# Huiweizhou/GCGCN

Measured on AMD Instinct MI355X. Metric: docs/sec fwd+bwd through CAGGC+MAGGC, higher is better.
Workload: dtype f32; 1 GPU; c2: GraphHops fwd+bwd, B=32/GPU N=64 D=256 L=2 H=8, train mode, E1/E2/X/params require grad, rotating inputs: 3 resident batches (805 MB of E per GPU), step i runs on batch i mod 3; global_batch=32, mode=graph, input_sets=3, parallelism=dp1, grad_allreduce=one coalesced collective after backward

## Files before the change

gcgcn_amd/_lib.py:

```python
from __future__ import annotations

import ctypes
import os
from ctypes import c_char_p, c_float, c_int, c_int64, c_uint64, c_void_p

_HERE = os.path.dirname(os.path.abspath(__file__))
LIB_PATH = os.environ.get("GCGCN_LIB") or os.path.join(_HERE, "lib", "libgcgcn_hip.so")

ABI_VERSION = 7

SALT_GAT = 0x47415431
SALT_MHA = 0x4D484131
SALT_GCN = 0x47434E31
SALT_GLUE = 0x474C5531

P = c_void_p
I = c_int
F = c_float
L = c_int64

class MhaHook(ctypes.Structure):
    _fields_ = [("flat_q", c_void_p), ("Q", c_void_p), ("P", c_void_p), ("A", c_void_p), ("dQ", c_void_p), ("rng_snap", c_void_p),
                ("p", ctypes.c_float)]


class EdgeRide(ctypes.Structure):
    _fields_ = [("B", ctypes.c_int32), ("N", ctypes.c_int32), ("D", ctypes.c_int32),
                ("inp", c_void_p), ("n_valid", c_void_p), ("out", c_void_p)]


SIGNATURES = {
    "gcgcn_version": (I, []),
    "gcgcn_last_error": (c_char_p, []),
    "gcgcn_set_option": (I, [c_char_p, I]),
    "gcgcn_debug_spread": (I, [L, L, L, L, P, P]),
    "gcgcn_debug_chain_plan": (I, [I] * 11 + [P]),
    "gcgcn_debug_head_plan": (I, [I, I, I, I, P]),
    "gcgcn_debug_gemm_plan": (I, [I, P, P, I, L, L, P]),
    "gcgcn_debug_edge_plan": (I, [I] * 13 + [P]),
    "gcgcn_debug_attn_plan": (I, [I] * 8 + [P]),
    "gcgcn_debug_out_bwd_plan": (I, [I] * 12 + [P]),
    "gcgcn_prof_start": (I, [c_char_p, I]),
    "gcgcn_prof_enable": (I, [I]),
    "gcgcn_prof_stop": (I, [P, P, P]),
    "gcgcn_rng_next": (I, [P, P, I, P]),
    "gcgcn_dropout_keep": (I, [P, L, P, c_uint64, F, P]),
    "gcgcn_dropout": (I, [P, P, L, P, c_uint64, F, P]),
    "gcgcn_gat_layout": (I, [I, I, P]),
    "gcgcn_gat_fwd": (I, [I, I, I, I, P, P, P, P, P, F, P, P, P, P, P, P, P, I, P, I, P]),
    "gcgcn_gat_bwd_scratch": (L, [I, I, I]),
    "gcgcn_gat_bwd": (I, [I, I, I, I, P, P, P, P, P, F, P, P, P, P, P, P, P, P, P, P, P, P, P, P, P]),
    "gcgcn_edge_mean_fwd": (I, [I, I, I, P, P, P, P]),
    "gcgcn_edge_mean_bwd": (I, [I, I, I, P, P, P, P]),
    "gcgcn_mha_layout": (I, [I, P]),
    "gcgcn_mha_scratch": (L, [I, I, I]),
    "gcgcn_row_blocks_ints": (L, [I, I]),
    "gcgcn_row_blocks": (I, [I, I, P, P, P]),
    "gcgcn_mha_fwd": (I, [I, I, I, I, P, P, P, P, F, P, P, P, P, P, P]),
    "gcgcn_mha_bwd": (I, [I, I, I, I, P, P, P, F, P, P, P, P, P, P, P, P, P, P, I, P, P]),
    "gcgcn_maggc_fusable": (I, [I, I, I]),
    "gcgcn_gcn_layout": (I, [I, I, I, P]),
    "gcgcn_gcn_scratch": (L, [I, I, I, I]),
    "gcgcn_gcn_fwd": (I, [I, I, I, I, I, P, P, P, P, P, P, F, P, F, P, P, P, P, P, P, P, P, P, P, P, P]),
    "gcgcn_gcn_bwd": (I, [I, I, I, I, I, P, P, P, P, P, P, F, P, F, P, P, P, P, P, P, P, P, P, P, P, P, P, P, P, P, P, P, P, P, P, P]),
    "gcgcn_defer_create": (P, []),
    "gcgcn_defer_destroy": (None, [P]),
    "gcgcn_defer_count": (I, [P]),
    "gcgcn_defer_flush": (I, [P, P]),
    "gcgcn_graphconv_fwd": (I, [I, I, I, I, I, P, P, P, P, P, P, P, P, P, P, P]),
    "gcgcn_graphconv_bwd": (I, [I, I, I, I, I, P, P, P, P, P, P, P, P, P, P, P, P, P, P, P, P, P, P, P, P]),
    "gcgcn_pair_bce_fwd": (I, [I, I, I, P, P, P, P, P, P]),
    "gcgcn_pair_bce_bwd": (I, [I, I, I, P, P, P, P, P, P]),
    "gcgcn_eval_ws_bytes": (L, [L, L]),
    "gcgcn_eval_scan": (I, [I, I, I, P, P, P, P, P, P, L, P, P]),
    "gcgcn_eval_rank": (I, [P, L, P, L, P, P]),
    "gcgcn_eval_curve": (I, [P, L, L, P, ctypes.c_double, P, P, P, P, P, L, P]),
    "gcgcn_producer_layout": (I, [I, I, P]),
    "gcgcn_producer_count": (I, [I, I, I, I, P, P, P, P]),
    "gcgcn_producer_sizes": (I, [I, I, I, I, I, I, I, L, L, P]),
    "gcgcn_producer_fwd": (I, [I, I, I, I, I, I, I, P, P, P, P, I, P, P, P, P, L, L, P, P, P, L, P, P]),
    "gcgcn_producer_bwd": (I, [I, I, I, I, I, I, I, P, P, P, P, I, P, P, P, P, L, L, P, P, P, P, P, P, P, P, P, P]),
    "gcgcn_edge_mean_fwd_compact": (I, [I, I, I, P, P, P, P, P, P]),
    "gcgcn_edge_mean_bwd_compact": (I, [I, I, I, P, P, P, P, P, P, P]),
    "gcgcn_gat_fwd_compact": (I, [I, I, I, I, P, P, P, P, P, P, P, F, P, P, P, P, P, P, P, I, I, P]),
    "gcgcn_gat_bwd_compact_scratch": (L, [I, I, I]),
    "gcgcn_gat_bwd_compact": (I, [I, I, I, I, P, P, P, P, P, P, P, F, P, P, P, P, P, P, P, P, P, P, P, P, P, P, P]),
    "gcgcn_head_layout": (I, [I, I, I, I, I, P]),
    "gcgcn_head_sizes": (I, [I, I, I, I, P]),
    "gcgcn_head_fwd": (I, [I, I, I, I, I, I, I, I, I, P, P, P, P, P, P, P, P, P, P, P]),
    "gcgcn_head_bwd": (I, [I, I, I, I, I, I, I, I, I, P, P, P, P, P, P, P, P, P, P, P, P, P, P, P, P]),
    "gcgcn_tensorise": (I, [I, I, I, I, I, I, I, P, I, P, I, P, I, P, P, P, P, P, P, P, P, P, P, P, P]),
    "gcgcn_adam_step": (I, [I, P, L, ctypes.c_double, ctypes.c_double, ctypes.c_double, P]),
    "gcgcn_adam_ws_bytes": (L, [I, L]),
    "gcgcn_adam_step_dev": (I, [I, P, L, ctypes.c_double, ctypes.c_double, ctypes.c_double, P, ctypes.c_double, P, L, P, P]),
    "gcgcn_gemm": (I, [I, I, I, P, L, I, P, L, I, P, L, I, L, L, L, F, P, I, I, I, I, P, L, P]),
    "gcgcn_gemm_dyn": (I, [I, I, I, P, L, I, P, L, I, P, L, P, I, P, I, L, P, L, P]),
    "gcgcn_lstm_ws_bytes": (L, [I] * 5),
    "gcgcn_lstm_fwd": (I, [I] * 5 + [P] * 10),
    "gcgcn_lstm_bwd": (I, [I] * 5 + [P] * 17 + [L, P]),
    "gcgcn_frontend_ws_bytes": (L, [I] * 9),
    "gcgcn_embed_fwd": (I, [I] * 8 + [P] * 9),
    "gcgcn_embed_bwd": (I, [I] * 8 + [P] * 5 + [I, I] + [P] * 4 + [L, P]),
    "gcgcn_context_fwd": (I, [I] * 5 + [P] * 8),
    "gcgcn_context_bwd": (I, [I] * 5 + [P] * 11 + [L, P]),
}

_lib = None


def lib() -> ctypes.CDLL:
    global _lib
    if _lib is None:
        if not os.path.exists(LIB_PATH):
            raise RuntimeError(
                f"gcgcn_amd: {LIB_PATH} not found. Build it with `make -C gcgcn_amd/csrc` "
                "(or `python -c 'import __graft_entry__ as g; g.build()'`). There is no CPU fallback.")
        handle = ctypes.CDLL(LIB_PATH)
        for name, (res, args) in SIGNATURES.items():
            fn = getattr(handle, name)
            fn.restype = res
            fn.argtypes = args
        if handle.gcgcn_version() != ABI_VERSION:
            raise RuntimeError(f"gcgcn_amd: ABI version {handle.gcgcn_version()} != {ABI_VERSION}")
        _lib = handle
    return _lib


def call(name: str, *args):
    h = lib()
    rc = getattr(h, name)(*args)
    if rc != 0:
        raise RuntimeError(f"{name} failed ({rc}): {h.gcgcn_last_error().decode()}")


def layout(kind: str, *dims) -> list:
    n = {"gat": 9, "mha": 3, "gcn": 7, "producer": 17, "head": 7}[kind]
    out = (c_int64 * n)()
    call(f"gcgcn_{kind}_layout", *dims, ctypes.cast(out, c_void_p))
    return list(out)
```

gcgcn_amd/csrc/api.hip:

```cpp
#include "../../include/gcgcn.h"

#include <stdarg.h>
#include <string.h>

#include <new>
#include <vector>

#include <stdlib.h>

#include "attn_plan.hpp"
#include "compact.hpp"
#include "gat_body.hpp"
#include "gemm.hpp"
#include "lstm.hpp"
#include "frontend.hpp"
#include "rowops.hpp"

namespace gc {

static thread_local char g_err[512] = "";

void set_error(const char* fmt, ...) {
  va_list ap;
  va_start(ap, fmt);
// ... 102 lines not shown
      o.value = value, o.resolved = true;
      return true;
    }
  return false;
}

static AttnQuery make_attn_query(int N, int D, int H, const void* Q, const void* dQ, bool hook, bool chain_attends, bool core_done) {
  return AttnQuery{N, D, H, attn_misalign(Q, dQ), hook, chain_attends, core_done, option("mha_core", 1)};
}

static int make_ride(const char* who, const gcgcn_edge_ride* ride, int kind, EdgeRide& r) {
  memset(&r, 0, sizeof(r));
  if (!ride) return 0;
  GC_REQUIRE(ride->B > 0 && ride->N > 0 && ride->D > 0 && ride->in && ride->out, "%s: bad edge ride B=%d N=%d D=%d", who,
             ride->B, ride->N, ride->D);
  GC_REQUIRE((long)ride->B * ride->N <= 0x3fffffffL, "%s: edge ride too large", who);
  r.kind = kind, r.B = ride->B, r.N = ride->N, r.D = ride->D;
  r.in = ride->in, r.n_valid = ride->n_valid, r.out = ride->out;
  return 0;
}

static void use_rows(GemmArgs& g, const int* rowblk, int mode, int zero_dead = 0) {
  if (!rowblk) return;
  g.rb = rowblk + ROWBLK_HDR, g.rb_n = rowblk;
  g.rb_mode = mode, g.rb_zero = zero_dead;
}

static const int* live_rows(const int32_t* rowblk, int N, bool ragged) {
  return (rowblk && ragged && N % 16 == 0 && N >= 32) ? rowblk : nullptr;
}

static ChainQuery make_query(int B, int N, int D, int L, int H, const GcnLayout& y, const float* flat, bool ragged, bool scratch,
                             bool hook, const EdgeRide& ride, const void* A, const void* Pn, const void* Y) {
  ChainQuery q = ChainQuery();
  q.B = B, q.N = N, q.D = D, q.L = L, q.H = H, q.gh = y.gh;
  q.HD = (long)H * D, q.oWd = y.oWd, q.wd_head = y.wd_head, q.oWlin = y.oWlin;
  q.flat = flat, q.ragged = ragged, q.scratch = scratch, q.hook = hook, q.ride = ride;
  q.A = A, q.Pn = Pn, q.Y = Y;
  q.chain = option("chain", 1), q.chain_big = option("chain_big", 0), q.chain_t = option("chain_t", 1);
  return q;
}

static GcnCtx make_ctx(int B, int N, int D, int L, int H, const GcnLayout& y, const float* X, const float* A,
                       const float* flat, const int* n_valid, Drop drop) {
  GcnCtx c;
  memset(&c, 0, sizeof(c));
  c.B = B, c.N = N, c.D = D, c.L = L, c.H = H, c.gh = y.gh;
  c.HD = (long)H * D, c.oWd = y.oWd, c.wd_head = y.wd_head;
  c.X = X, c.A = A, c.flat = flat, c.n_valid = n_valid, c.drop = drop;
  return c;
}

struct EdgeOperand {
  const float* E;
  CmpE ce;
};

static int gat_node_fwd(const float* X, const float* flat, float* uvc, float* s, long M, int D, int Dh, int uvc_valid, void* rng_state,
                        void* rng_snaps, int rng_count, hipStream_t st) {
  if (!uvc_valid) {
    GC_TRY(gat_fold_fwd(flat, uvc, D, Dh, st, rng_state, rng_snaps, rng_count));
    return node_score_fwd(X, uvc, s, M, D, st);
  }
  return node_score_fwd(X, uvc, s, M, D, st, rng_state, rng_snaps, rng_count);
}

static int gat_bwd(const EdgeOperand& eo, int B, int N, int D, int Dh, const float* X, const int* n_valid, const float* flat, Drop drop,
                   const float* uvc, const float* P, const float* dA, const float* dEbar, const float* dX_in, float* dX, float* dE,
                   float* dbias, float* dflat, float* dlogit, float* ds, float* dvpart, float* duvc, float* scratch, DeferQueue* dq,
                   hipStream_t st) {
  const bool compact = eo.E == nullptr;
  const long M = (long)B * N;
  const float* v = uvc + D;
  const EdgePlan plan = edge_plan_bwd({B, N, D, compact, true, dE != nullptr, dEbar != nullptr,
                                       compact ? 0u : edge_misalign(eo.E, v, dE, dEbar, nullptr)});
  const GatTail tail{P, dA, uvc, dX_in, ds, dX, drop, B, plan.slices};
  if (plan.route == EdgePlan::ONE) {
    GC_TRY(gat_dlogit(P, dA, uvc, dX_in, dlogit, ds, dX, B, N, D, plan.slices, drop, st));
  } else if (plan.route == EdgePlan::THREE) {
    GC_TRY(softmax_bwd(P, dA, dlogit, M, N, drop, st));
    GC_TRY(colsum(dlogit, nullptr, ds, N, N, N, B, (long)N * N, 0, N, 0, nullptr, st));
    GC_TRY(node_score_bwd(ds, uvc, dX_in, dX, M, D, st));
  }
  if (compact)
    GC_TRY(cmp_bwd(eo.ce, v, n_valid, dlogit, dEbar, dE, dvpart, scratch + plan.rowbuf_off, dbias, plan, B, N, D, st));
  else
    GC_TRY(edge_bwd(eo.E, v, n_valid, dlogit, dEbar, dE, dvpart, plan, B, N, D, st, dq, &tail));
  long part_off[3];
  int ns = 0;
  GC_TRY(colsum3(X, ds, duvc, M, D, D, dvpart, nullptr, duvc + D, M, D, D, ds, nullptr, duvc + 2 * D, M, 1, 1, scratch,
                 st, false, part_off, &ns));
  return gat_fold_bwd(flat, duvc, dflat, D, Dh, st, scratch, part_off, ns);
}

static OutBwdPlan out_bwd_plan(const OutBwdQuery& q) {
  OutBwdPlan p = OutBwdPlan();
  const bool masked = q.ragged || q.odrop;
  if (q.fuse) {
    p.mask = masked ? OutBwdPlan::MASK_CHAIN : OutBwdPlan::MASK_NONE;
    p.wsum = q.H == 1 ? OutBwdPlan::WSUM_NONE : q.wsum_fwd ? OutBwdPlan::WSUM_FORWARD : OutBwdPlan::WSUM_HERE;
    p.dwlin = OutBwdPlan::DWLIN_BACK;
    const bool in_chain = 2 * q.B <= COL_RIDE_SLICES;
    p.col1 = in_chain ? OutBwdPlan::COL1_CHAIN : OutBwdPlan::COL1_BACK;
    p.chain_slices = in_chain ? 2 * q.B : 0;
    return p;
  }
  p.mask = masked ? OutBwdPlan::MASK_LAUNCH : OutBwdPlan::MASK_NONE;
  constexpr long fold_max = 2L << 20;
  const bool fold = q.scratch && (q.H == 1 || q.wsum_fwd) && (long)q.B * q.N * q.H * q.D <= fold_max && q.dxres_aligned;
  p.fold = !fold ? OutBwdPlan::FOLD_NONE : q.H == 1 ? OutBwdPlan::FOLD_ONE_HEAD : OutBwdPlan::FOLD_HEADS;
  p.fold_drop = fold && (q.H == 1 || q.drop);
  p.head_sum_launch = !fold;
  p.wsum = p.fold == OutBwdPlan::FOLD_HEADS ? OutBwdPlan::WSUM_FORWARD : OutBwdPlan::WSUM_NONE;
  p.dwlin = OutBwdPlan::DWLIN_FRONT;
  p.col1 = q.scratch ? OutBwdPlan::COL1_FRONT : OutBwdPlan::COL1_OWN_LAUNCH;
  return p;
}

static OutBwdCol2 out_bwd_plan_col2(const OutBwdPlan& p, bool front_reduced) {
  switch (p.col1) {
    case OutBwdPlan::COL1_OWN_LAUNCH: return {OutBwdCol2::DONE, 0};
    case OutBwdPlan::COL1_CHAIN: return {OutBwdCol2::BACK_LAUNCH, p.chain_slices};
    case OutBwdPlan::COL1_BACK: return {OutBwdCol2::BACK_REDUCE, 0};
    default: break;
  }
  if (front_reduced) return {OutBwdCol2::FRONT_REDUCE, 0};
  if (p.head_sum_launch) return {OutBwdCol2::HEAD_SUM_KERNEL, 0};
  return {OutBwdCol2::BACK_LAUNCH, COL_RIDE_SLICES};
}

}

using namespace gc;

extern "C" {

int gcgcn_version(void) { return 7; }
const char* gcgcn_last_error(void) { return g_err; }

int gcgcn_set_option(const char* name, int value) {
  GC_REQUIRE(name, "set_option: null name");
  if (set_opt(name, value)) return 0;
  set_error("set_option: unknown option '%s'", name);
  return 1;
}

int64_t gcgcn_row_blocks_ints(int B, int N) { return (B > 0 && N > 0 && N % 16 == 0) ? row_blocks_ints(B, N) : 0; }
int gcgcn_row_blocks(int B, int N, const int32_t* n_valid, int32_t* out, void* stream) {
  return row_blocks(n_valid, B, N, out, (hipStream_t)stream);
}

int gcgcn_prof_start(const char* kernel_prefix, int capacity) {
  GC_REQUIRE(kernel_prefix && capacity > 0, "prof_start: bad arguments");
  for (hipEvent_t e : g_prof.ev) (void)hipEventDestroy(e);
  g_prof.ev.assign(2 * (size_t)capacity, nullptr);
  for (auto& e : g_prof.ev) {
    if (hipEventCreate(&e) != hipSuccess) {
      set_error("prof_start: hipEventCreate failed");
      return 2;
    }
  }
  strncpy(g_prof.filter, kernel_prefix, sizeof(g_prof.filter) - 1);
  g_prof.used = 0;
  g_prof.work = 0;
  g_prof.on = true;
  return 0;
}
int gcgcn_prof_enable(int on) {
  g_prof.on = on != 0 && !g_prof.ev.empty();
  return 0;
}
int gcgcn_prof_stop(double* total_ms, int* launches, double* work) {
  GC_REQUIRE(total_ms && launches, "prof_stop: null pointer");
  if (work) *work = g_prof.work;
// ... 136 lines not shown
  o[2] = o[1] + D;
  return 0;
}

int gcgcn_mha_fwd(int B, int N, int D, int H, const float* X, const int32_t* n_valid, const float* flat,
                  const void* rng_snap, float p, float* Q, float* P, float* A, float* scratch, const int32_t* rowblk, void* stream) {
  hipStream_t st = (hipStream_t)stream;
  GC_TRY(check_dims("mha_fwd", B, N, D, 1, H));
  const long wse = scratch ? gemm_scratch_elems(B, N, D, 1) : 0;
  GC_REQUIRE(X && flat && Q && P, "mha_fwd: null pointer");
  const AttnPlan plan = attn_plan_fwd(make_attn_query(N, D, H, Q, nullptr, false, false, false));
  const GcnCtx::MhaFwd m = attn_core(GcnCtx::MhaFwd{Q, P, A}, D, H, plan, rng_snap, p);
  GC_REQUIRE(!m.drop.snap || A, "mha_fwd: dropout on but A is NULL");
  const long M = (long)B * N;
  {
    GemmArgs g = gemm_nt(X, D, flat, D, Q, D, (int)M, D, D).split_ws(scratch, wse);
    g.bias = flat + (long)D * D;
    use_rows(g, live_rows(rowblk, N, n_valid != nullptr), 1, 1);
    GC_TRY(gemm(g, st));
  }
  switch (plan.route) {
    case AttnPlan::CORE: return mha_core_fwd(m, n_valid, B, N, D, H, st);
    default: {
      GemmArgs g = gemm_nt(Q, D, Q, D, P, N, N, N, m.dh).split_ws(scratch, wse);
      g.batch_z1(B, (long)N * D, (long)N * D, (long)H * N * N).batch_z2(H, m.dh, m.dh, (long)N * N);
      g.alpha = m.alpha;
      GC_TRY(gemm(g, st));
      return softmax_fwd(P, nullptr, n_valid, P, A, M * H, N, H, m.drop, st);
    }
  }
}

int64_t gcgcn_mha_scratch(int B, int N, int D) { return scratch_elems(B, N, D, 1); }

int gcgcn_mha_bwd(int B, int N, int D, int H, const float* X, const float* flat, const void* rng_snap, float p,
                  const float* Q, const float* P, const float* dA, const float* dX_in, float* dX, float* dflat, float* dS,
                  float* dQ, float* scratch, void* defer_queue, int core_done, const int32_t* rowblk, void* stream) {
  hipStream_t st = (hipStream_t)stream;
  GC_TRY(check_dims("mha_bwd", B, N, D, 1, H));
  const long wse = scratch ? gemm_scratch_elems(B, N, D, 1) : 0;
  GC_REQUIRE(X && flat && Q && P && dA && dX && dflat && dS && dQ, "mha_bwd: null pointer");
  const AttnPlan plan = attn_plan_bwd(make_attn_query(N, D, H, Q, dQ, false, false, core_done != 0));
  const MhaPass mp = attn_core(mha_pass(Q, P, dA, dQ, B, N, D, H), D, H, plan, rng_snap, p);
  const long M = (long)B * N;
  switch (plan.route) {
    case AttnPlan::DONE: break;
    case AttnPlan::CORE: GC_TRY(mha_core_bwd(mp, st)); break;
    default:
      GC_TRY(softmax_bwd(P, dA, dS, M * H, N, mp.drop, st));
      for (int pass = 0; pass < 2; ++pass) {
        GemmArgs g = (pass == 0 ? gemm_nn : gemm_tn)(dS, N, Q, D, dQ, D, N, mp.dh, N).split_ws(scratch, wse);
        g.batch_z1(B, (long)H * N * N, (long)N * D, (long)N * D).batch_z2(H, (long)N * N, mp.dh, mp.dh);
        g.alpha = mp.alpha, g.accumulate = pass;
        GC_TRY(gemm(g, st));
      }
  }
  {
    GemmArgs gs[2] = {gemm_nn(dQ, D, flat, D, dX, D, (int)M, D, D).split_ws(scratch, wse),
                      gemm_tn(dQ, D, X, D, dflat, D, D, D, (int)M).split_ws(scratch, wse)};
    gs[0].add = dX_in, gs[0].ldadd = D;
    const int* rows = live_rows(rowblk, N, true);
    use_rows(gs[0], rows, 1, 1), use_rows(gs[1], rows, 2);
    const int ng = gemm_defer((DeferQueue*)defer_queue, gs[1]) ? 1 : 2;
    if (scratch) {
      const ColRide cr = col_sum(dQ, M, D, D, dflat + (long)D * D, scratch + wse);
      bool later = false;
      GC_TRY(gemm_group(gs, ng, st, &cr, (ng == 1 && defer_queue) ? &later : nullptr));
      if (later) {
        const ColRide c2 = cr.stage2(COL_RIDE_SLICES);
        if (!gemm_defer_col2((DeferQueue*)defer_queue, c2)) GC_TRY(col_sum_stage2_launch(c2, st));
      }
    } else {
      GC_TRY(gemm_group(gs, ng, st));
      GC_TRY(colsum(dQ, nullptr, dflat + (long)D * D, M, D, D, 1, 0, 0, 0, 0, scratch, st));
    }
  }
  return 0;
}

void* gcgcn_defer_create(void) { return new (std::nothrow) DeferQueue(); }
void gcgcn_defer_destroy(void* queue) { delete (DeferQueue*)queue; }
int gcgcn_defer_count(const void* queue) { return queue ? ((const DeferQueue*)queue)->n + ((const DeferQueue*)queue)->ncol2 : 0; }
int gcgcn_defer_flush(void* queue, void* stream) { return gemm_flush_deferred((DeferQueue*)queue, (hipStream_t)stream); }

int gcgcn_pair_bce_fwd(int B, int N, int R, const float* logits, const float* labels, const int32_t* n_valid, float* loss,
                       float* part, void* stream) {
  GC_REQUIRE(B > 0 && N > 0 && R > 0 && (long)B * N <= 0x7fffffffL && (long)N * R <= 0x7fffffffL,
             "pair_bce_fwd: bad shape B=%d N=%d R=%d", B, N, R);
  GC_REQUIRE(logits && labels && loss && part, "pair_bce_fwd: null pointer");
  return pair_bce_fwd(logits, labels, n_valid, loss, part, B, N, R, (hipStream_t)stream);
}

int gcgcn_pair_bce_bwd(int B, int N, int R, const float* logits, const float* labels, const int32_t* n_valid,
                       const float* dloss, float* dlogits, void* stream) {
  GC_REQUIRE(B > 0 && N > 0 && R > 0, "pair_bce_bwd: bad shape B=%d N=%d R=%d", B, N, R);
  GC_REQUIRE(logits && labels && dlogits, "pair_bce_bwd: null pointer");
  return pair_bce_bwd(logits, labels, n_valid, dloss, dlogits, B, N, R, (hipStream_t)stream);
}

int gcgcn_gcn_layout(int D, int L, int H, int64_t* o) {
  GC_TRY(check_dims("gcn_layout", 1, 1, D, L, H));
  GC_REQUIRE(o, "gcn_layout: null pointer");
  const GcnLayout y = gcn_layout(D, L, H);
  o[0] = y.oWnX, o[1] = y.oWe, o[2] = y.oWd, o[3] = y.oWlin, o[4] = y.oblin, o[5] = y.total, o[6] = y.wd_head;
  return 0;
}

int gcgcn_gcn_fwd(int B, int N, int D, int L, int H, const float* X, const float* Ebar, const float* A,
                  const int32_t* n_valid, const float* flat, const void* rng_snap, float p, const void* out_rng_snap,
                  float out_p, float* out, float* Pn, float* Y, float* HO, float* rinv, float* G, float* wsum, float* scratch,
                  const gcgcn_edge_ride* ride, const gcgcn_mha_hook* mha, const int32_t* rowblk, void* stream) {
  hipStream_t st = (hipStream_t)stream;
  GC_TRY(check_dims("gcn_fwd", B, N, D, L, H));
  AttnQuery aq = make_attn_query(N, D, H, mha ? mha->Q : nullptr, nullptr, mha != nullptr, false, false);
  const int refusal = attn_hook_refusal(aq);
  GC_REQUIRE(refusal != ATTN_REFUSED_SHAPE, "gcn_fwd: attention hook on a shape it does not serve");
  GC_REQUIRE(!mha || (mha->flat_q && mha->Q && mha->P), "gcn_fwd: attention hook on a shape it does not serve");
  GC_REQUIRE(refusal != ATTN_REFUSED_ALIGN, "gcn_fwd: attention hook: misaligned Q");
  if (mha) A = mha->A ? mha->A : mha->P;
  EdgeRide er;
  GC_TRY(make_ride("gcn_fwd", ride, 1, er));
  const long wse = scratch ? gemm_scratch_elems(B, N, D, H) : 0;
  GC_REQUIRE(X && Ebar && A && flat && out && Pn && Y && HO && rinv && G, "gcn_fwd: null pointer");
  const GcnLayout y = gcn_layout(D, L, H);
  const Drop drop = make_drop(rng_snap, GCGCN_SALT_GCN, p);
  const long M = (long)B * N;
  const long HD = (long)H * D;
  GC_REQUIRE(M <= 0x7fffffffL, "gcn_fwd: B*N too large");
  ChainQuery q = make_query(B, N, D, L, H, y, flat, n_valid != nullptr, scratch != nullptr, mha != nullptr, er, A, Pn, Y);
  q.G = G, q.HO = HO, q.X = X;
  const ChainPlan plan = chain_plan_fwd(q);
  aq.chain_attends = plan.attention;
  const AttnPlan ap = attn_plan_fwd(aq);
  GcnCtx c = make_ctx(B, N, D, L, H, y, X, A, flat, n_valid, drop);
  c.G = G, c.Pn = Pn, c.Y = Y, c.HO = HO, c.rinv = rinv;
  if (plan.ride) c.ride = er;
  const int* rows = live_rows(rowblk, N, n_valid != nullptr);

  {
    GemmArgs g3[3] = {gemm_nn(X, D, flat + y.oWnX, HD, Pn, HD, (int)M, (int)HD, D).split_ws(scratch, wse),
                      gemm_nn(Ebar, D, flat + y.oWe, HD, G, HD, (int)M, (int)HD, D).split_ws(scratch, wse), GemmArgs()};
    const int ng = mha ? 3 : 2;
    if (mha) {
      g3[2] = gemm_nt(X, D, mha->flat_q, D, mha->Q, D, (int)M, D, D).split_ws(scratch, wse);
      g3[2].bias = mha->flat_q + (long)D * D;
    }
    for (int q = 0; q < ng; ++q) use_rows(g3[q], rows, 1, 1);
    const ColRide hs = head_sum(flat + y.oWlin, H, D, wsum);
    GC_TRY(gemm_group(g3, ng, st, (wsum && H > 1) ? &hs : nullptr));
  }
  {
    if (er.kind && !plan.ride) {
      GC_TRY(edge_fwd(er.in, nullptr, er.n_valid, er.out, nullptr, nullptr, nullptr, Drop(), er.B, er.N, er.D, st));
      er.kind = 0;
    }
    if (mha) {
      const GcnCtx::MhaFwd m = attn_core(GcnCtx::MhaFwd{mha->Q, mha->P, mha->A}, D, H, ap, mha->rng_snap, mha->p);
      GC_REQUIRE(!m.drop.snap || mha->A, "gcn_fwd: attention dropout on but A is NULL");
      switch (ap.route) {
        case AttnPlan::CHAIN: c.mha = m; break;
        default: GC_TRY(mha_core_fwd(m, n_valid, B, N, D, H, st));
      }
    }
    if (plan.kind != ChainPlan::NONE) {
      GC_TRY(gcn_chain_fwd(c, plan, st));
    } else {
// ... 206 lines not shown
    GemmArgs g = gemm_tn(A, N, dS, Dout, dT, Dout, N, Dout, N).batch_z1(B, (long)N * N, (long)N * Dout, (long)N * Dout);
    GC_TRY(gemm(g, st, 0, 1));
  }
  GemmArgs gs[5] = {
      gemm_nt(dS, Dout, T, Dout, dA, N, N, N, Dout).batch_z1(B, (long)N * Dout, (long)N * Dout, (long)N * N),
      gemm_tn(Ebar, De, dS, Dout, dWe, Dout, De, Dout, (int)M),
      gemm_nt(dS, Dout, We, Dout, dEbar, De, (int)M, De, Dout),
      gemm_tn(X, Din, dT, Dout, dWn, Dout, Din, Dout, (int)M),
      gemm_nt(dT, Dout, Wn, Dout, dX, Din, (int)M, Din, Dout)};
  for (auto& g : gs) g.split_ws(scratch, wse);
  gs[0].rowadd = drow, gs[0].sRa1 = N;
  GC_TRY(gemm_group(gs, 5, st));
  return 0;
}

int gcgcn_debug_spread(int64_t n_tiles, int64_t n_others, int64_t cohort, int64_t pct, int32_t* kind, int32_t* ordinal) {
  GC_REQUIRE(n_tiles >= 0 && n_others >= 0 && kind && ordinal, "debug_spread: bad arguments");
  const Spread sp = make_spread(n_tiles, n_others, cohort, pct);
  for (long x = 0; x < n_tiles + n_others; ++x) {
    int idx = -1;
    kind[x] = spread_pick((int)x, sp, idx) ? 1 : 0;
    ordinal[x] = idx;
  }
  return 0;
}

int gcgcn_debug_chain_plan(int bwd, int B, int N, int D, int L, int H, int ragged, int ride, int hook, int scratch, int misalign,
                           int32_t* out) {
  GC_TRY(check_dims("debug_chain_plan", B, N, D, L, H));
  GC_REQUIRE(out, "debug_chain_plan: null pointer");
  int slot = 0;
  auto at = [&](int bit) { return (const float*)(uintptr_t)(0x100000ul * ++slot + ((misalign & bit) ? 4 : 0)); };
  EdgeRide er = EdgeRide();
  if (ride) er.kind = bwd ? 2 : 1, er.B = B, er.N = N, er.D = D, er.in = at(4), er.out = const_cast<float*>(at(4));
  ChainQuery q = make_query(B, N, D, L, H, gcn_layout(D, L, H), at(8), ragged != 0, scratch != 0, hook != 0, er, at(1), at(1), at(1));
  q.G = at(1), q.HO = at(1), q.X = at(1), q.dYa = at(1), q.dM = at(1), q.dP = at(1), q.dA = at(1);
  q.dout = at(2), q.dXres = at(2), q.dout_m = at(2);
  const ChainPlan p = bwd ? chain_plan_bwd(q) : chain_plan_fwd(q);
  out[0] = p.kind, out[1] = p.aligned, out[2] = p.full, out[3] = p.fuse, out[4] = p.attention, out[5] = p.ride;
  return 0;
}

int gcgcn_debug_out_bwd_plan(int fuse, int B, int N, int D, int H, int scratch, int wsum_fwd, int ragged, int odrop, int drop,
                             int dxres_misaligned, int front_reduced, int32_t* out) {
  GC_REQUIRE(B > 0 && N > 0 && D > 0 && H > 0 && out, "debug_out_bwd_plan: bad arguments");
  GC_REQUIRE(!fuse || scratch, "debug_out_bwd_plan: the fused chain backward without scratch");
  const OutBwdPlan p = out_bwd_plan({fuse != 0, B, N, D, H, scratch != 0, wsum_fwd != 0, ragged != 0, odrop != 0, drop != 0, !dxres_misaligned});
  const OutBwdCol2 c2 = out_bwd_plan_col2(p, front_reduced != 0);
  out[0] = p.mask, out[1] = p.wsum, out[2] = p.fold, out[3] = p.fold_drop, out[4] = p.head_sum_launch, out[5] = p.dwlin, out[6] = p.col1;
  out[7] = p.chain_slices, out[8] = c2.where, out[9] = c2.back_ready_slices;
  return 0;
}

int gcgcn_debug_attn_plan(int bwd, int N, int D, int H, int hook, int chain_attends, int core_done, int misalign, int32_t* out) {
  GC_REQUIRE(N > 0 && D > 0 && H > 0 && D % H == 0 && out, "debug_attn_plan: bad arguments");
  const void *Q = (const void*)(uintptr_t)(0x100000ul + ((misalign & 1) ? 4 : 0)), *dQ = (const void*)(uintptr_t)(0x200000ul + ((misalign & 2) ? 4 : 0));
  const AttnQuery q = make_attn_query(N, D, H, Q, bwd ? dQ : nullptr, hook != 0, chain_attends != 0, core_done != 0);
  const AttnPlan p = bwd ? attn_plan_bwd(q) : attn_plan_fwd(q);
  out[3] = attn_hook_refusal(q);
  out[0] = out[3] ? -1 : p.route, out[1] = out[3] ? -1 : p.kchunk, out[2] = p.fusable;
  return 0;
}

int gcgcn_debug_edge_plan(int pass, int compact, int B, int N, int D, int ragged, int att, int has_dE, int has_dEbar, int misalign,
                          int parked_tiles, int any_rb, int col_C, int32_t* out) {
  (void)ragged;
  GC_REQUIRE(pass >= 0 && pass <= 2 && B > 0 && N > 0 && D > 0 && parked_tiles >= 0 && col_C >= 0 && out, "debug_edge_plan: bad arguments");
  GC_REQUIRE((long)B * N * 9 + parked_tiles < (1L << 31) && (long)B * N * D < (1L << 31), "debug_edge_plan: shape too large");
  GC_REQUIRE(!compact || D <= 64 * CMAXK, "debug_edge_plan: hidden width %d (compact rows support up to %d)", D, 64 * CMAXK);
  const bool dense_bwd = pass == 1 && !compact;
  GC_REQUIRE(!dense_bwd || att, "debug_edge_plan: a dense backward without a logit gradient is pass 2");
  const EdgeQuery q = {B, N, D, compact != 0, att != 0, has_dE != 0, has_dEbar != 0, (unsigned)misalign};
  EdgePlan p = pass == 0 ? edge_plan_fwd(q) : pass == 1 ? edge_plan_bwd(q) : edge_plan_bcast(q);
  if (dense_bwd && p.carry_ok) edge_plan_carry(p, parked_tiles, any_rb != 0, col_C);
  const int na = -1;
  out[0] = p.compact ? na : p.vec, out[1] = p.att, out[2] = p.route, out[3] = p.slices, out[4] = dense_bwd ? p.ngat : na;
  out[5] = (int)p.lds, out[6] = p.lds_limit ? (int)p.lds_ok() : na, out[7] = dense_bwd ? (int)p.carry_ok : na, out[8] = dense_bwd ? (int)p.RB : na;
  out[9] = (int)p.grid, out[10] = dense_bwd ? p.col_base : na, out[11] = dense_bwd ? p.ncolwg : na;
  out[12] = dense_bwd ? p.spread.na : na, out[13] = dense_bwd ? p.spread.cohort : na, out[14] = dense_bwd ? p.spread.stride : na;
  out[15] = (int)p.scratch, out[16] = (int)p.rowbuf_off;
  return 0;
}

static const int64_t kEvalMaxRecords = 0xffffffffLL;

int64_t gcgcn_eval_ws_bytes(int64_t n_records, int64_t n_keep) {
  if (n_records < 0 || n_keep < 0 || n_records > kEvalMaxRecords) {
    set_error("eval: %lld records do not fit the 32-bit ordinal of a record (at most %lld)", (long long)n_records,
              (long long)kEvalMaxRecords);
    return -1;
  }
  return eval_ws_bytes(n_records, n_keep < n_records ? n_keep : n_records);
}

int gcgcn_eval_scan(int B, int N, int R, const float* logits, const float* labels, const uint8_t* in_train, const int32_t* n_valid,
                    const int64_t* doc_base, uint64_t* records, int64_t capacity, int64_t* counters, void* stream) {
  GC_REQUIRE(B > 0 && N > 0 && R > 1 && (long)B * N <= 0x7fffffffL && (long)N * R <= 0x7fffffffL,
             "eval_scan: bad shape B=%d N=%d R=%d", B, N, R);
  GC_REQUIRE(logits && labels && doc_base && records && counters, "eval_scan: null pointer");
  GC_REQUIRE(capacity > 0 && capacity <= kEvalMaxRecords, "eval_scan: capacity %lld outside (0, %lld]: a record's ordinal has 32 bits",
             (long long)capacity, (long long)kEvalMaxRecords);
  return eval_scan(logits, labels, in_train, n_valid, doc_base, records, capacity, counters, B, N, R, (hipStream_t)stream);
}

int gcgcn_eval_rank(const uint64_t* records, int64_t n, void* ws, int64_t ws_bytes, int64_t* sorted_off, void* stream) {
  GC_REQUIRE(n > 0 && n <= kEvalMaxRecords, "eval_rank: %lld records outside (0, %lld]", (long long)n, (long long)kEvalMaxRecords);
  GC_REQUIRE(records && ws && sorted_off, "eval_rank: null pointer");
  return eval_rank(records, n, ws, ws_bytes, sorted_off, (hipStream_t)stream);
}

int gcgcn_eval_curve(const uint64_t* ranked, int64_t m, int64_t n_records, const int64_t* counters, double input_theta,
                     float* pr_x, float* pr_y, float* ign_pr_y, double* result, void* ws, int64_t ws_bytes, void* stream) {
  GC_REQUIRE(m > 0 && m <= n_records && n_records <= kEvalMaxRecords, "eval_curve: bad sizes m=%lld n_records=%lld", (long long)m,
             (long long)n_records);
  GC_REQUIRE(ranked && counters && pr_x && pr_y && result && ws, "eval_curve: null pointer");
  return eval_curve(ranked, m, counters, input_theta, pr_x, pr_y, ign_pr_y, result, ws, ws_bytes, n_records, (hipStream_t)stream);
}

int gcgcn_gemm(int M, int N, int K, const float* A, int64_t lda, int a_kc, const float* B, int64_t ldb, int b_kc,
               float* C, int64_t ldc, int batch, int64_t sA, int64_t sB, int64_t sC, float alpha, const float* bias,
               int relu, int accumulate, int tile, int splits, float* ws, int64_t ws_elems, void* stream) {
  GemmArgs g = gemm_stored(a_kc, b_kc, A, lda, B, ldb, C, ldc, M, N, K).batch_z2(batch, sA, sB, sC).split_ws(ws, ws_elems);
  g.alpha = alpha, g.bias = bias, g.relu = relu, g.accumulate = accumulate;
  return gemm(g, (hipStream_t)stream, tile, splits);
}


int gcgcn_gemm_dyn(int M, int N, int K, const float* A, int64_t lda, int a_kc, const float* B, int64_t ldb, int b_kc, float* C,
                   int64_t ldc, const float* bias, int accumulate, const int32_t* count, int dyn, int64_t cap, float* ws,
                   int64_t ws_elems, void* stream) {
  GemmArgs g = gemm_stored(a_kc, b_kc, A, lda, B, ldb, C, ldc, M, N, K).split_ws(ws, ws_elems);
  g.bias = bias, g.accumulate = accumulate;
  return gemm_dyn(g, count, dyn, cap, (hipStream_t)stream);
}

static int lstm_shape_ok(const char* who, int B, int T, int I, int H, int nd) {
  GC_REQUIRE(H == LSTM_H, "%s: hidden width %d is not served (the recurrence kernels hold H = %d)", who, H, LSTM_H);
  GC_REQUIRE(nd == 1 || nd == 2, "%s: %d directions (1 or 2)", who, nd);
  GC_REQUIRE(B >= 1 && T >= 1 && I >= 1, "%s: bad shape B=%d T=%d I=%d", who, B, T, I);
  GC_REQUIRE((long)B * T * nd * 4 * H <= 0x7fffffffL && (long)B * T * I <= 0x7fffffffL, "%s: B=%d T=%d I=%d is too large", who, B, T, I);
  return 0;
}

int64_t gcgcn_lstm_ws_bytes(int B, int T, int I, int H, int nd) {
  if (lstm_shape_ok("lstm_ws_bytes", B, T, I, H, nd)) return -1;
  return (int64_t)sizeof(float) * lstm_ws_elems(B, T, I, nd);
}

int gcgcn_lstm_fwd(int B, int T, int I, int H, int nd, const float* x, const float* w_ih, const float* w_hh, const float* bias,
                   const float* h0, const float* c0, float* out, float* gates, float* csave, void* stream) {
  GC_TRY(lstm_shape_ok("lstm_fwd", B, T, I, H, nd));
  GC_REQUIRE(x && w_ih && w_hh && bias && h0 && c0 && out && gates, "lstm_fwd: null pointer");
  GC_REQUIRE((((uintptr_t)w_hh) & 15) == 0, "lstm_fwd: w_hh must be 16-byte aligned");
  return lstm_fwd(B, T, I, nd, x, w_ih, w_hh, bias, h0, c0, out, gates, csave, (hipStream_t)stream);
}

int gcgcn_lstm_bwd(int B, int T, int I, int H, int nd, const float* x, const float* w_ih, const float* w_hh, const float* h0,
                   const float* c0, const float* out, const float* gates, const float* csave, const float* dout, float* dgates,
                   float* dx, float* dw_ih, float* dw_hh, float* db, float* dh0, float* dc0, void* ws, int64_t ws_bytes, void* stream) {
  GC_TRY(lstm_shape_ok("lstm_bwd", B, T, I, H, nd));
  GC_REQUIRE(x && w_ih && w_hh && h0 && c0 && out && gates && csave && dout && dgates && dx && dw_ih && dw_hh && db && dh0 && dc0 && ws,
             "lstm_bwd: null pointer");
  GC_REQUIRE(dout != out, "lstm_bwd: dout aliases the output (H_prev is read from the output after dout has been consumed)");
  GC_REQUIRE(dgates != gates, "lstm_bwd: dgates aliases the saved gates");
  GC_REQUIRE((((uintptr_t)ws) & 15) == 0 && (((uintptr_t)out) & 15) == 0 && (((uintptr_t)h0) & 15) == 0,
             "lstm_bwd: ws, out and h0 must be 16-byte aligned");
// ... 94 lines not shown
```

gcgcn_amd/csrc/edge.hip:

```cpp
#include <string.h>

#include "edge_body.hpp"
#include "compact.hpp"
#include "gat_body.hpp"
#include "gemm_body.hpp"
#include "rowops.hpp"

namespace gc {

template <int VEC, bool ATT>
__global__ __launch_bounds__(64 * EW) void edge_fwd_kernel(const float* __restrict__ E, const float* __restrict__ v,
                                                           const int* __restrict__ n_valid, float* __restrict__ Ebar,
                                                           const float* __restrict__ coladd, float* __restrict__ P,
                                                           float* __restrict__ Aout, Drop drop, int N, int D,
                                                           const unsigned char* __restrict__ mask) {
  extern __shared__ __attribute__((aligned(16))) float cs[];
  edge_fwd_row<VEC, ATT, EW>(E, v, n_valid, Ebar, coladd, P, Aout, drop, N, D, blockIdx.x, cs, mask);
}

template <int VEC>
__device__ __forceinline__ void edge_bwd_row(const float* __restrict__ E, const float* __restrict__ v,
                                             const int* __restrict__ n_valid, const float* __restrict__ dlogit,
                                             const float* __restrict__ dEbar, float* __restrict__ dE,
                                             float* __restrict__ dvpart, int N, int D, int nt, const int bi,
                                             float* __restrict__ sm, const GatTail& gt) {
  float* dl = sm;
  float* cs = sm + ((N + 3) & ~3);
  const int b = bi / N, i = bi - b * N;
  const int t = threadIdx.x, lane = t & 63, wave = t >> 6;
  const int nv = n_valid ? min(max(n_valid[b], 0), N) : N;
  float* dEr = dE ? dE + (long)bi * N * D : nullptr;
  float* dvp = dvpart + (long)bi * D;
  if (i >= nv) {
    for (int c = t; c < D; c += 64 * EW) dvp[c] = 0.f;
    if (dEr) {
      const long tot = (long)N * D;
      for (long o = t; o < tot; o += 64 * EW) dEr[o] = 0.f;
    }
    return;
  }
  if (gt.P) {
    if (wave == 0) {
      const long o = (long)bi * N + min(lane, N - 1);
      float p = gt.P[o], g = gt.dA[o];
      if (lane >= N) p = 0.f, g = 0.f;
      if (gt.drop.snap) g = (rng_u32(drop_key(gt.drop), (uint64_t)((long)bi * N + lane)) >= gt.drop.thresh) ? g * gt.drop.scale : 0.f;
      const float dot = wave_sum(g * p);
      if (lane < N) dl[lane] = p * (g - dot);
    }
  } else {
    for (int j = t; j < N; j += 64 * EW) dl[j] = dlogit[(long)bi * N + j];
  }
  __syncthreads();
  const float* __restrict__ Er = E + (long)bi * N * D;
  const float inv = 1.f / (float)nv;
  const int nchunk = (D + 64 * VEC - 1) / (64 * VEC);
  for (int q = 0; q < nchunk; ++q) {
    const int c = (q * 64 + lane) * VEC;
    const bool act = c < D;
    float vr[VEC], g[VEC], acc[VEC];
#pragma unroll
    for (int e = 0; e < VEC; ++e) vr[e] = 0.f, g[e] = 0.f, acc[e] = 0.f;
    if (act) {
      vload<VEC>(vr, v + c);
      if (dEbar) {
        vload<VEC>(g, dEbar + (long)bi * D + c);
#pragma unroll
        for (int e = 0; e < VEC; ++e) g[e] *= inv;
      }
    }
    int j = wave;
    for (; j + (EUNR - 1) * EW < nv; j += EUNR * EW) {
      float x[EUNR][VEC];
#pragma unroll
      for (int u = 0; u < EUNR; ++u) {
#pragma unroll
        for (int e = 0; e < VEC; ++e) x[u][e] = 0.f;
        if (act) vload_nt<VEC>(x[u], Er + (long)(j + u * EW) * D + c);
      }
#pragma unroll
      for (int u = 0; u < EUNR; ++u) {
        const float d = dl[j + u * EW];
        float o[VEC];
// ... 19 lines not shown
        acc[e] = fmaf(d, x[e], acc[e]);
        o[e] = fmaf(d, vr[e], g[e]);
      }
      if (dEr && act) {
        if (nt) vstore_nt<VEC>(dEr + (long)j * D + c, o);
        else vstore<VEC>(dEr + (long)j * D + c, o);
      }
    }
    if (dEr && act) {
      float z[VEC];
#pragma unroll
      for (int e = 0; e < VEC; ++e) z[e] = 0.f;
      for (int jj = nv + wave; jj < N; jj += EW) vstore<VEC>(dEr + (long)jj * D + c, z);
    }
    if (act) vstore<VEC>(cs + wave * D + c, acc);
  }
  __syncthreads();
  for (int c = t; c < D; c += 64 * EW) {
    float s = 0.f;
#pragma unroll
    for (int w = 0; w < EW; ++w) s += cs[w * D + c];
    dvp[c] = s;
  }
}

template <int VEC>
__global__ __launch_bounds__(64 * EW) void edge_bwd_kernel(const float* __restrict__ E, const float* __restrict__ v,
                                                           const int* __restrict__ n_valid,
                                                           const float* __restrict__ dlogit,
                                                           const float* __restrict__ dEbar, float* __restrict__ dE,
                                                           float* __restrict__ dvpart, int N, int D, int nt,
                                                           const GatTail gt) {
  extern __shared__ __attribute__((aligned(16))) float sm[];
  const int ngat = gt.P ? gt.B * gt.slices : 0;
  if ((int)blockIdx.x < ngat) {
    const int b = blockIdx.x / gt.slices;
    gat_dlogit_doc(gt.P, gt.dA, gt.uvc, gt.dXin, nullptr, gt.ds, gt.dX, N, D, gt.drop, b, blockIdx.x - b * gt.slices, gt.slices, sm);
    return;
  }
  edge_bwd_row<VEC>(E, v, n_valid, dlogit, dEbar, dE, dvpart, N, D, nt, blockIdx.x - ngat, sm, gt);
}

template <int VEC, bool RB>
__global__ __launch_bounds__(64 * EW) void edge_bwd_carry_kernel(const float* __restrict__ E, const float* __restrict__ v,
                                                                 const int* __restrict__ n_valid,
                                                                 const float* __restrict__ dlogit,
                                                                 const float* __restrict__ dEbar, float* __restrict__ dE,
                                                                 float* __restrict__ dvpart, int N, int D, int nt,
                                                                 const Spread sp, const GatTail gt, const GemmGroup gg,
                                                                 const int col_base) {
  __shared__ __attribute__((aligned(16))) float tile_lds[lds_floats<1, 1, true, true>()];
  int r;
  if (col_base > 0 && (int)blockIdx.x >= col_base) {
    col_ride_stage2_block(gg.col, (int)blockIdx.x - col_base);
    return;
  }
  if (spread_pick((int)blockIdx.x, sp, r)) {
    gemm_group_block<RB>(gg, r, tile_lds);
    return;
  }
  const int ngat = gt.P ? gt.B * gt.slices : 0;
  if (r < ngat) {
    const int b = r / gt.slices;
    gat_dlogit_doc(gt.P, gt.dA, gt.uvc, gt.dXin, nullptr, gt.ds, gt.dX, N, D, gt.drop, b, r - b * gt.slices, gt.slices, tile_lds);
    return;
  }
  edge_bwd_row<VEC>(E, v, n_valid, dlogit, dEbar, dE, dvpart, N, D, nt, r - ngat, tile_lds, gt);
}

template <int VEC>
__global__ __launch_bounds__(64 * EW) void edge_bcast_kernel(const float* __restrict__ dEbar,
                                                             const int* __restrict__ n_valid, float* __restrict__ dE,
                                                             int N, int D, int nt) {
  edge_bcast_row<VEC, EW>(dEbar, n_valid, dE, N, D, nt, blockIdx.x);
}

static inline bool al16(const void* p) { return (((uintptr_t)p) & 15) == 0; }
unsigned edge_misalign(const void* E, const void* v, const void* dE, const void* dEbar, const void* Ebar) {
  return (al16(E) ? 0 : EDGE_MIS_E) | (al16(v) ? 0 : EDGE_MIS_V) | (al16(dE) ? 0 : EDGE_MIS_DE) | (al16(dEbar) ? 0 : EDGE_MIS_DEBAR) |
         (al16(Ebar) ? 0 : EDGE_MIS_EBAR);
}
constexpr size_t EDGE_LDS_MAX = 160 * 1024;
constexpr size_t CMP_LDS_MAX = 64 * 1024;
constexpr size_t TILE_LDS = sizeof(float) * lds_floats<1, 1, true, true>();
static_assert(sizeof(float) * GAT_DOC_LDS <= TILE_LDS, "GAT passenger needs more LDS than a tile");

static EdgePlan plan_rows(const EdgeQuery& q, unsigned operands) {
  EdgePlan p;
  p.compact = q.compact, p.att = q.att;
  p.vec = (!q.compact && q.D % 4 == 0 && !(q.mis & operands)) ? 4 : 1;
  p.grid = (long)q.B * q.N;
  return p;
}

EdgePlan edge_plan_fwd(const EdgeQuery& q) {
  EdgePlan p = plan_rows(q, EDGE_MIS_E | EDGE_MIS_EBAR | (q.att ? EDGE_MIS_V : 0));
  p.lds = ((size_t)(q.compact ? CW4 : EW) * q.D + (q.att ? (size_t)q.N : 0)) * sizeof(float);
  p.lds_limit = q.compact ? CMP_LDS_MAX : EDGE_LDS_MAX;
  return p;
}

EdgePlan edge_plan_bwd(const EdgeQuery& q) {
  EdgePlan p = plan_rows(q, EDGE_MIS_E | EDGE_MIS_V | (q.has_dE ? EDGE_MIS_DE : 0) | (q.has_dEbar ? EDGE_MIS_DEBAR : 0));
  if (q.att) {
    p.route = q.N > GT ? EdgePlan::THREE : (q.compact ? EdgePlan::ONE : EdgePlan::RIDE);
    if (p.route != EdgePlan::THREE) p.slices = gat_dlogit_slices(q.D);
    if (p.route == EdgePlan::RIDE) p.ngat = q.B * p.slices;
    const long a = colsum_scratch_elems((long)q.B * q.N, q.D, 1), b = 3L * 64 * (2 * q.D + 1);
    p.scratch = a > b ? a : b;
    if (q.compact) p.rowbuf_off = p.scratch, p.scratch += 2L * q.B * q.N;
  }
  if (q.compact) {
    p.lds = ((size_t)CW4 * q.D + 2 * CW4) * sizeof(float);
    return p;
  }
  const size_t lds_row = ((size_t)((q.N + 3) & ~3) + (size_t)EW * q.D) * sizeof(float);
  p.lds = (p.ngat && lds_row < sizeof(float) * GAT_DOC_LDS) ? sizeof(float) * GAT_DOC_LDS : lds_row;
  p.lds_limit = EDGE_LDS_MAX;
  p.carry_ok = p.vec == 4 && lds_row <= TILE_LDS;
  p.grid += p.ngat;
  return p;
}

EdgePlan edge_plan_bcast(const EdgeQuery& q) {
  if (!q.compact) return plan_rows(q, EDGE_MIS_DE | EDGE_MIS_DEBAR);
  EdgeQuery m = q;
  m.att = false;
  return edge_plan_bwd(m);
}

void edge_plan_carry(EdgePlan& p, int ntile, bool any_rb, int col_C) {
  if (ntile <= 0) return;
  const long rows = p.grid;
  p.ntile = ntile, p.RB = any_rb;
  p.ncolwg = col_C > 0 ? cdiv(col_C, 256) : 0;
  p.col_base = col_C > 0 ? (int)(rows + ntile) : 0;
  p.grid = rows + ntile + p.ncolwg;
  constexpr int spread_pct = 90, cohort = 256, spread_min = 1024;
  p.spread = make_spread(ntile, rows, cohort, ntile >= spread_min ? spread_pct : 0);
  p.lds = 0;
}

constexpr int NT_STORE = 0;

int edge_fwd(const float* E, const float* v, const int* n_valid, float* Ebar, const float* coladd, float* P, float* A,
             Drop drop, int B, int N, int D, hipStream_t st, const unsigned char* mask) {
  GC_REQUIRE(E && Ebar, "edge_fwd: null pointer");
  GC_REQUIRE(B > 0 && N > 0 && D > 0, "edge_fwd: bad shape B=%d N=%d D=%d", B, N, D);
  const bool att = P != nullptr;
  GC_REQUIRE(!att || (v && coladd), "edge_fwd: attention requested without v / node scores");
  const EdgePlan p = edge_plan_fwd({B, N, D, false, att, false, false, edge_misalign(E, v, nullptr, nullptr, Ebar)});
  GC_REQUIRE(p.lds_ok(), "edge_fwd: N=%d D=%d needs %zu B of LDS", N, D, p.lds);
  dim3 grid((unsigned)p.grid), block(64 * EW);
  const char* tag = att ? "edge_fwd_att" : "edge_fwd_mean";
  const double bytes = 4.0 * B * N * N * D;
#define GC_EDGE_FWD(V, AT) \
  GC_LAUNCH_TIMED(tag, bytes, (edge_fwd_kernel<V, AT>), grid, block, p.lds, st, E, v, n_valid, Ebar, coladd, P, A, drop, N, D, mask)
  if (p.vec == 4) {
    if (att) GC_EDGE_FWD(4, true);
    else GC_EDGE_FWD(4, false);
  } else {
    if (att) GC_EDGE_FWD(1, true);
    else GC_EDGE_FWD(1, false);
  }
#undef GC_EDGE_FWD
  return check_launch("edge_fwd");
}

int edge_bwd(const float* E, const float* v, const int* n_valid, const float* dlogit, const float* dEbar, float* dE,
             float* dvpart, const EdgePlan& plan, int B, int N, int D, hipStream_t st, DeferQueue* carry, const GatTail* tail) {
  GatTail gt;
  memset(&gt, 0, sizeof gt);
  if (tail && plan.route == EdgePlan::RIDE) gt = *tail;
  GC_REQUIRE(E && v && (dlogit || gt.P) && dvpart, "edge_bwd: null pointer");
  GC_REQUIRE(!gt.P || (N <= GT && gt.B == B && gt.slices == plan.slices && gt.dA && gt.uvc && gt.ds && gt.dX), "edge_bwd: bad GAT passenger");
  GC_REQUIRE(!plan.compact && plan.ngat == (gt.P ? B * gt.slices : 0) &&
                 (plan.vec == 4) == (D % 4 == 0 && !edge_misalign(E, v, dE, dEbar, nullptr)),
             "edge_bwd: the plan was made for other operands");
  static_assert(sizeof(GatTail) + sizeof(GemmGroup) + 96 <= 4096, "edge_bwd_carry_kernel: kernel arguments exceed 4 KB");
  GC_REQUIRE(plan.lds_ok(), "edge_bwd: N=%d D=%d needs %zu B of LDS", N, D, plan.lds);
  EdgePlan p = plan;
  dim3 block(64 * EW);
  const double bytes = (dE ? 8.0 : 4.0) * B * N * N * D;
  GemmGroup gg;
  double gflops = 0;
  const int ntile = (p.carry_ok && carry && carry->n > 0) ? gemm_take_deferred(carry, gg, &gflops) : 0;
  if (ntile > 0) {
    const bool col = gemm_take_deferred_col2(carry, gg.col);
    bool any_rb = false;
    for (int i = 0; i < gg.nprob; ++i) any_rb = any_rb || gg.p[i].rb != nullptr;
    edge_plan_carry(p, ntile, any_rb, col ? gg.col.C : 0);
    dim3 grid((unsigned)p.grid);
#define GC_EDGE_CARRY(RBV)                                                                                                  \
  GC_LAUNCH_TIMED("edge_bwd", bytes, (edge_bwd_carry_kernel<4, RBV>), grid, block, 0, st, E, v, n_valid, dlogit, dEbar, dE, \
                  dvpart, N, D, NT_STORE, p.spread, gt, gg, p.col_base)
    if (p.RB) GC_EDGE_CARRY(true);
    else GC_EDGE_CARRY(false);
#undef GC_EDGE_CARRY
    return check_launch("edge_bwd_carry");
  }
  dim3 grid((unsigned)p.grid);
#define GC_EDGE_BWD(V)                                                                                                             \
  GC_LAUNCH_TIMED("edge_bwd", bytes, (edge_bwd_kernel<V>), grid, block, p.lds, st, E, v, n_valid, dlogit, dEbar, dE, dvpart, N, D, \
                  NT_STORE, gt)
  if (p.vec == 4) GC_EDGE_BWD(4);
  else GC_EDGE_BWD(1);
#undef GC_EDGE_BWD
  return check_launch("edge_bwd");
}

int edge_bcast(const float* dEbar, const int* n_valid, float* dE, int B, int N, int D, hipStream_t st) {
  GC_REQUIRE(dEbar && dE, "edge_bcast: null pointer");
  const EdgePlan p = edge_plan_bcast({B, N, D, false, false, true, true, edge_misalign(nullptr, nullptr, dE, dEbar, nullptr)});
  dim3 grid((unsigned)p.grid), block(64 * EW);
  ProfScope ps("edge_bcast", st, 4.0 * B * N * N * D);
  if (p.vec == 4) hipLaunchKernelGGL((edge_bcast_kernel<4>), grid, block, 0, st, dEbar, n_valid, dE, N, D, NT_STORE);
  else hipLaunchKernelGGL((edge_bcast_kernel<1>), grid, block, 0, st, dEbar, n_valid, dE, N, D, NT_STORE);
  return check_launch("edge_bcast");
}

}
```

gcgcn_amd/csrc/edge_plan.hpp:

```cpp
#pragma once
#include "common.hpp"

namespace gc {

enum EdgeMisalign { EDGE_MIS_E = 1, EDGE_MIS_V = 2, EDGE_MIS_DE = 4, EDGE_MIS_DEBAR = 8, EDGE_MIS_EBAR = 16 };
unsigned edge_misalign(const void* E, const void* v, const void* dE, const void* dEbar, const void* Ebar);

struct EdgeQuery {
  int B, N, D;
  bool compact;
  bool att;
  bool has_dE, has_dEbar;
  unsigned mis;
};

struct EdgePlan {
  enum Route { RIDE = 0, ONE = 1, THREE = 2 };
  bool compact = false, att = false;
  int vec = 1;
  int route = -1;
  int slices = -1;
  int ngat = 0;
  size_t lds = 0;
  size_t lds_limit = 0;
  bool lds_ok() const { return lds_limit == 0 || lds <= lds_limit; }
  bool carry_ok = false;
  int ntile = 0, ncolwg = 0, col_base = 0;
  bool RB = false;
  long grid = 0;
  Spread spread = {0, 0, 0};
  long scratch = -1;
  long rowbuf_off = -1;
};

EdgePlan edge_plan_fwd(const EdgeQuery& q);
EdgePlan edge_plan_bwd(const EdgeQuery& q);
EdgePlan edge_plan_bcast(const EdgeQuery& q);
void edge_plan_carry(EdgePlan& p, int ntile, bool any_rb, int col_C);

}
```

gcgcn_amd/csrc/gemm.hip:

```cpp
#include <stdlib.h>

#include "attn_plan.hpp"
#include "edge_body.hpp"
#include "gemm_body.hpp"
#include "mha_body.hpp"
#include "rowops.hpp"

namespace gc {

template <int TM, int TN, bool AKC, bool BKC, bool ALIGNED, bool RB = false>
__global__ __launch_bounds__(256, (TM * TN == 4 ? 2 : 1)) void gemm_kernel(const GemmArgs g) {
  __shared__ __attribute__((aligned(16))) float lds[lds_floats<TM, TN, AKC, BKC>()];
  const int gx = gridDim.x, gy = gridDim.y;
  const int nwg = gx * gy * gridDim.z;
  const int q = blockIdx.x + gx * (blockIdx.y + gy * blockIdx.z);
  if (RB && g.rb && g.rb_mode == 1) {
    int bx, by, zs, wide;
    if (!tile_of_rows(g, q, gx, gy, bx, by, zs, wide)) return;
    gemm_body<TM, TN, AKC, BKC, ALIGNED, GC_GEMM_EG, 0, EPI_ALL, PlainOperands, RB>(g, lds, bx, by, zs, threadIdx.x, true, PlainOperands(), nullptr, 0, wide);
    return;
  }
  const int b = xcd_remap(q, nwg);
  gemm_body<TM, TN, AKC, BKC, ALIGNED, GC_GEMM_EG, 0, EPI_ALL, PlainOperands, RB>(g, lds, b % gx, (b / gx) % gy, b / (gx * gy));
}

__device__ __forceinline__ void col_ride_stage1(const ColRide& cr, int cb, float* red) {
  const int lane = threadIdx.x & 63, wave = threadIdx.x >> 6;
  const int ncb = (cr.C + 63) >> 6;
  const int sp = cb / ncb, c = (cb - sp * ncb) * 64 + lane;
  const long rps = (cr.R + COL_RIDE_SLICES - 1) / COL_RIDE_SLICES;
  const long r0 = sp * rps, r1 = min(cr.R, r0 + rps);
  float acc = 0.f;
  if (c < cr.C) {
    long r = r0 + wave;
    for (; r + 28 < r1; r += 32) {
      float v[8];
#pragma unroll
      for (int u = 0; u < 8; ++u) v[u] = cr.X[(r + 4 * u) * cr.ld + c];
#pragma unroll
      for (int u = 0; u < 8; ++u) acc += v[u];
    }
    for (; r < r1; r += 4) acc += cr.X[r * cr.ld + c];
  }
  red[wave * 64 + lane] = acc;
  __syncthreads();
  if (wave == 0 && c < cr.C) cr.part[(long)sp * cr.C + c] = (red[lane] + red[64 + lane]) + (red[128 + lane] + red[192 + lane]);
}

__device__ __forceinline__ void group_tail(const GemmGroup& gg, const int idx, float* __restrict__ lds) {
  const ColRide& cr = gg.col;
  if (cr.ready_slices < 0) {
    const int e = idx * 256 + threadIdx.x;
    if (e < cr.C) {
      const int ld = (int)cr.ld, H = (int)cr.R, k = e / ld, c = e - k * ld;
      float s = 0.f;
      for (int h0 = 0; h0 < H; h0 += 8) {
        float v[8];
#pragma unroll
        for (int u = 0; u < 8; ++u) v[u] = cr.X[((long)k * H + min(h0 + u, H - 1)) * ld + c];
#pragma unroll
        for (int u = 0; u < 8; ++u) s += (h0 + u < H) ? v[u] : 0.f;
      }
      cr.out[e] = s;
    }
    return;
  }
  if (cr.ready_slices > 0) {
    col_ride_stage2_block(cr, idx);
    return;
  }
  col_ride_stage1(cr, idx, lds);
}

template <bool RB>
__global__ __launch_bounds__(256, 4) void gemm_group_kernel(const GemmGroup gg) {
  __shared__ __attribute__((aligned(16))) float lds[lds_floats<1, 1, true, true>()];
  const int tiles = gg.tile_begin[gg.nprob];
  if ((int)blockIdx.x >= tiles) {
    group_tail(gg, blockIdx.x - tiles, lds);
    return;
  }
  gemm_group_block<RB>(gg, blockIdx.x, lds);
}

template <bool RB>
__global__ __launch_bounds__(256, 4) void gemm_group_pass_kernel(const GemmGroup gg, const MhaPass mp) {
  __shared__ __attribute__((aligned(16))) float lds[lds_floats<1, 1, true, true>()];
  const int tiles = gg.tile_begin[gg.nprob], inter = tiles + mp.count;
  const int x = blockIdx.x;
  if (x >= inter) {
    group_tail(gg, x - inter, lds);
    return;
  }
  const int before = (int)((long)x * mp.count / inter);
  if ((int)((long)(x + 1) * mp.count / inter) > before) {
    mha_core_bwd_body(lds, before, mp.Q, mp.P, mp.dA, mp.dQ, mp.N, mp.D, mp.H, mp.dh, mp.kchunk, mp.alpha, mp.drop);
    return;
  }
  gemm_group_block<RB>(gg, x - before, lds);
}

__device__ __forceinline__ void reduce4(const GemmArgs& g, int z, long idx4) {
  const long mn = (long)g.M * g.N;
  const long idx = idx4 * 4;
  if (idx >= mn) return;
  const long nb = (long)g.batch1 * g.batch2;
  int row = (int)(idx / g.N);
  const int col = (int)(idx - (long)row * g.N);
  const int z1 = z / g.batch2, z2 = z - z1 * g.batch2;
  int nsplit = g.splits;
  if (g.rb && g.rb_mode == 1) {
    const int bi = row >> 4;
    const int prow = g.rb[bi] * 16 + (row & 15);
    const int tm = (g.M + 63) >> 6;
    nsplit *= split_width(g, min((*g.rb_n + 3) >> 2, tm), tm);
    if (bi >= *g.rb_n) {
      if (g.rb_zero) {
        const float4 zero = make_float4(0.f, 0.f, 0.f, 0.f);
        float* c = g.C + z1 * g.sC1 + z2 * g.sC2 + (long)prow * g.ldc + col;
        c[0] = 0.f, c[1] = 0.f, c[2] = 0.f, c[3] = 0.f;
        if (g.C2) {
          float* c2 = g.C2 + z1 * g.sC21 + z2 * g.sC22 + (long)prow * g.ldc2 + col;
          c2[0] = zero.x, c2[1] = zero.y, c2[2] = zero.z, c2[3] = zero.w;
        }
      }
      return;
    }
    row = prow;
  }
  const float4* w = reinterpret_cast<const float4*>(g.ws + (long)z * mn + idx);
  const long stride4 = nb * mn / 4;
  float4 acc = make_float4(0.f, 0.f, 0.f, 0.f);
  if (nsplit <= 4) {
    for (int s = 0; s < nsplit; ++s) {
      const float4 v = w[(long)s * stride4];
      acc.x += v.x, acc.y += v.y, acc.z += v.z, acc.w += v.w;
    }
  } else {
    for (int s0 = 0; s0 < nsplit; s0 += 8) {
      float4 v[8];
#pragma unroll
      for (int u = 0; u < 8; ++u) v[u] = w[(long)min(s0 + u, nsplit - 1) * stride4];
#pragma unroll
      for (int u = 0; u < 8; ++u)
        if (s0 + u < nsplit) acc.x += v[u].x, acc.y += v[u].y, acc.z += v[u].z, acc.w += v[u].w;
    }
  }
  if (!(g.add || g.bias || g.rowadd || g.rowscale || g.relu || g.accumulate || g.n_valid || g.C2) && g.alpha == 1.f) {
    float* c = g.C + z1 * g.sC1 + z2 * g.sC2 + (long)row * g.ldc + col;
    if ((((uintptr_t)c) & 15) == 0) {
      *reinterpret_cast<float4*>(c) = acc;
    } else {
      c[0] = acc.x, c[1] = acc.y, c[2] = acc.z, c[3] = acc.w;
    }
    return;
  }
  const Epi e = make_epi(g, z1, z2);
  epi_store4(g, e, row, col, acc);
}

__global__ __launch_bounds__(256) void splitk_reduce_group_kernel(const GemmGroup gg) {
  int b = blockIdx.x, i = 0;
  if (b >= gg.red_begin[gg.nprob]) {
    const ColRide& cr = gg.col;
    const int c = (b - gg.red_begin[gg.nprob]) * 256 + threadIdx.x;
    if (c < cr.C) {
      float s = 0.f;
      for (int q = 0; q < COL_RIDE_SLICES; ++q) s += cr.part[(long)q * cr.C + c];
      cr.out[c] = s;
    }
    return;
  }
  while (i + 1 < gg.nprob && b >= gg.red_begin[i + 1]) ++i;
  b -= gg.red_begin[i];
  const GemmArgs& g = gg.p[i];
  if (g.splits <= 1) return;
  const int per = (int)(((long)g.M * g.N / 4 + 255) / 256);
  const int z = b / per;
  reduce4(g, z, (long)(b - z * per) * 256 + threadIdx.x);
}

__global__ __launch_bounds__(256) void splitk_reduce_kernel(const GemmArgs g) {
  reduce4(g, blockIdx.y, (long)blockIdx.x * 256 + threadIdx.x);
}

int splitk_reduce(const GemmArgs& g, hipStream_t st, const char* what) {
  ProfScope ps("gemm_splitk_reduce", st);
  dim3 rgrid(cdiv((long)g.M * g.N / 4, 256), g.batch1 * g.batch2);
  hipLaunchKernelGGL(splitk_reduce_kernel, rgrid, dim3(256), 0, st, g);
  return check_launch(what);
}

static inline bool aligned16(const void* p) { return (((uintptr_t)p) & 15) == 0; }
static long tiles_of(const GemmArgs& g) { return (long)cdiv(g.M, 64) * cdiv(g.N, 64) * g.batch1 * g.batch2; }
static long work_of(const GemmArgs& g) { return tiles_of(g) * cdiv(g.K, BK); }
static double flops_of(const GemmArgs& g) { return 2.0 * g.M * g.N * g.K * g.batch1 * g.batch2; }

static int pick_splits(int K, long work) {
  constexpr int thr_pct = 250;
  const long iters = cdiv(K, BK);
  long thr = work / 1024 * thr_pct / 100;
  if (thr < 8) thr = 8;
  int splits = 1;
  while (iters / splits > thr && splits < 16 && K % (splits * 2 * BK) == 0) splits *= 2;
  return splits;
}
static int dyn_splits(long tiles, long cap) {
  long want = (1024 + tiles - 1) / tiles, most = cap / (8 * BK);
  if (most < 1) most = 1;
  const long splits = want < most ? want : most;
  return (int)(splits > 64 ? 64 : splits);
}
static bool ws_holds(const GemmArgs& g, long slabs) { return g.ws && slabs * g.M * g.N <= g.ws_elems && g.N % 4 == 0 && aligned16(g.ws); }

enum GemmForm {
  GEMM_SINGLE,
  GEMM_MEMBER,
  GEMM_PARK,
  GEMM_DYN_M,
  GEMM_DYN_K
};
struct GemmPlan {
  bool ok;
  bool interior;
  int splits, ksplit, widen;
  int rb_mode;
  long tiles;
  bool reduce;
  bool zero_fill;
  int grid;
};
static GemmPlan gemm_plan(GemmArgs& g, GemmForm form, int splits, long group_work, long cap) {
  GemmPlan p = {};
  const bool dyn = form == GEMM_DYN_M || form == GEMM_DYN_K;
  const long nb = (long)g.batch1 * g.batch2;
  if (dyn && nb != 1) { set_error("gemm_dyn: batched problems are not supported"); return p; }
  if (dyn && cap == 0) cap = 1;
  if (dyn) (form == GEMM_DYN_M ? g.M : g.K) = (int)((cap + 63) & ~63L);
  if (!(g.A && g.B && g.C)) { set_error("gemm: null operand"); return p; }
  if (!(g.M >= 0 && g.N >= 0 && g.K >= 1 && g.batch1 >= 1 && g.batch2 >= 1)) { set_error("gemm: bad shape"); return p; }
  {
    long ldmax = g.ldc;
    if (g.add && g.ldadd > ldmax) ldmax = g.ldadd;
    if (g.C2 && g.ldc2 > ldmax) ldmax = g.ldc2;
    if (g.add2 && g.ldadd2 > ldmax) ldmax = g.ldadd2;
    if ((long)g.M * ldmax >= (1L << 32)) { set_error("gemm: M * ld = %ld exceeds 32-bit epilogue offsets", (long)g.M * ldmax); return p; }
  }
  const bool widen_on = option("split_widen", 1) != 0;
  g.vecA = aligned16(g.A) && g.lda % 4 == 0 && g.sA1 % 4 == 0 && g.sA2 % 4 == 0;
  g.vecB = aligned16(g.B) && g.ldb % 4 == 0 && g.sB1 % 4 == 0 && g.sB2 % 4 == 0;
  p.tiles = tiles_of(g);
  if (form != GEMM_SINGLE) splits = form == GEMM_MEMBER ? 0 : 1;
  if (splits == 0) {
    splits = pick_splits(g.K, form == GEMM_MEMBER ? group_work : work_of(g));
    if (splits == 1 && g.rb && g.rb_mode == 1 && cdiv(g.K, BK) >= 48 && p.tiles <= 1024 && g.K % (2 * BK) == 0 && widen_on) splits = 2;
  }
  if (splits > 1 && !(ws_holds(g, splits * nb) && g.K % (splits * BK) == 0)) splits = 1;
  g.splits = splits;
  g.ksplit = (splits > 1) ? g.K / splits : g.K;
  p.interior = g.vecA && g.vecB && g.M % 64 == 0 && g.N % 64 == 0 && g.ksplit % BK == 0;
  if (g.rb) {
    const bool served = p.interior && g.rb_n && ((g.rb_mode == 1 && g.a_kc && nb == 1) ||
// ... 315 lines not shown
}

static const DynPairForm pair_wx = {"gemm_dyn_pair", 0, {2, 1}};
int gemm_dyn_pair(const GemmArgs& gw, const GemmArgs& gx, const int* cnt, long cap, hipStream_t st) { return dyn_pair(pair_wx, gw, gx, cnt, cap, st); }
static const DynPairForm pair_ww = {"gemm_dyn_pair_ww", 1, {2, 2}};
int gemm_dyn_pair_ww(const GemmArgs& ga, const GemmArgs& gb, const int* cnt, long cap, hipStream_t st) { return dyn_pair(pair_ww, ga, gb, cnt, cap, st); }
static const DynPairForm pair_xx = {"gemm_dyn_pair_xx", 2, {1, 1}};
int gemm_dyn_pair_xx(const GemmArgs& ga, const GemmArgs& gb, const int* cnt, long cap, hipStream_t st) { return dyn_pair(pair_xx, ga, gb, cnt, cap, st); }

bool gemm_defer(DeferQueue* q, const GemmArgs& g_in) {
  if (!q) return false;
  GemmArgs g = g_in;
  if (q->n >= DeferQueue::CAP || g.M == 0 || g.N == 0) return false;
  const GemmPlan p = gemm_plan(g, GEMM_PARK, 1, 0, 0);
  if (!(p.ok && p.interior)) return false;
  g.ws = nullptr, g.ws_elems = 0;
  q->done[q->n] = 0;
  q->p[q->n++] = g;
  return true;
}

bool gemm_defer_col2(DeferQueue* q, const ColRide& c) {
  if (!q || q->ncol2 >= DeferQueue::COLCAP || c.ready_slices <= 0 || !c.part || !c.out || c.C <= 0) return false;
  q->col2[q->ncol2++] = c;
  return true;
}
bool gemm_take_deferred_col2(DeferQueue* q, ColRide& out) {
  if (!q || q->ncol2 == 0) return false;
  out = q->col2[--q->ncol2];
  return true;
}

static void sort_parked(DeferQueue* q, bool small_first = false) {
  auto before = [&](const GemmArgs& a, int da, const GemmArgs& b, int db) {
    if (a.K != b.K) return a.K > b.K;
    return small_first && tiles_of(a) - da < tiles_of(b) - db;
  };
  for (int i = 1; i < q->n; ++i)
    for (int j = i; j > 0 && before(q->p[j], q->done[j], q->p[j - 1], q->done[j - 1]); --j) {
      const GemmArgs t = q->p[j];
      const int d = q->done[j];
      q->p[j] = q->p[j - 1], q->p[j - 1] = t;
      q->done[j] = q->done[j - 1], q->done[j - 1] = d;
    }
}

template <class G>
static int take_parked(DeferQueue* q, G& gg, double* flops, long max_tiles, bool small_first = false) {
  gg.nprob = 0;
  gg.tile_begin[0] = 0;
  if (!q || q->n == 0 || max_tiles <= 0) return 0;
  sort_parked(q, small_first);
  int wgs = 0, np = 0, keep = 0;
  for (int i = 0; i < q->n; ++i) {
    const GemmArgs& g = q->p[i];
    const int total = (int)tiles_of(g), avail = total - q->done[i];
    const long take = (np < G::MAXP && max_tiles > 0) ? (avail < max_tiles ? avail : max_tiles) : 0;
    if (take > 0) {
      wgs = (wgs + 7) & ~7;
      gg.tile_begin[np] = wgs, gg.tile_count[np] = total, gg.tile_first[np] = q->done[i], gg.tile_take[np] = (int)take;
      gg.red_begin[np] = 0;
      gg.p[np++] = g;
      wgs += (int)take;
      max_tiles -= take;
      if (flops) *flops += flops_of(g) * (double)take / total;
    }
    if (q->done[i] + take < total) {
      q->p[keep] = g, q->done[keep] = q->done[i] + (int)take;
      ++keep;
    }
  }
  q->n = keep;
  for (int i = keep; i < DeferQueue::CAP; ++i) q->done[i] = 0;
  gg.nprob = np;
  gg.tile_begin[np] = wgs, gg.red_begin[np] = 0;
  return wgs;
}

int gemm_take_deferred(DeferQueue* q, GemmGroup& gg, double* flops) { return take_parked(q, gg, flops, 1L << 40); }
int gemm_take_deferred_pairs(DeferQueue* q, GemmGroup4& gg, double* flops, long max_wgs, bool small_first) {
  return take_parked(q, gg, flops, max_wgs, small_first);
}

template <bool RB>
__global__ __launch_bounds__(256, 4) void gemm_parked_kernel(const GemmGroup gg) {
  __shared__ __attribute__((aligned(16))) float lds[lds_floats<1, 1, true, true>()];
  gemm_group_block<RB>(gg, blockIdx.x, lds);
}

int gemm_flush_deferred(DeferQueue* q, hipStream_t stream) {
  while (q && q->n > 0) {
    bool partial = false;
    for (int i = 0; i < q->n; ++i) partial = partial || q->done[i] > 0;
    if (partial) {
      GemmGroup gg;
      double fl = 0;
      const int wgs = gemm_take_deferred(q, gg, &fl);
      if (wgs > 0) {
        GC_LAUNCH_TIMED("gemm_group", fl, by_row_blocks(gg, gemm_parked_kernel<true>, gemm_parked_kernel<false>), dim3(wgs), dim3(256), 0, stream, gg);
        if (int e = check_launch("gemm_parked")) return e;
      }
      continue;
    }
    GemmArgs probs[GemmGroup::MAXP];
    const int n = q->n < GemmGroup::MAXP ? q->n : GemmGroup::MAXP;
    for (int i = 0; i < n; ++i) probs[i] = q->p[q->n - n + i];
    q->n -= n;
    if (int e = gemm_group(probs, n, stream)) return e;
  }
  ColRide c2;
  while (gemm_take_deferred_col2(q, c2))
    if (int e = col_sum_stage2_launch(c2, stream)) return e;
  return 0;
}

}

#include "../../include/gcgcn.h"

extern "C" {

int gcgcn_debug_gemm_plan(int form, const int64_t* prob_a, const int64_t* prob_b, int splits, int64_t group_work, int64_t cap, int32_t* out) {
  using namespace gc;
  GC_REQUIRE(form >= 0 && form <= 7 && prob_a && (form < 5 || prob_b) && cap >= 0 && out, "debug_gemm_plan: bad arguments");
  GC_REQUIRE(prob_a[0] > 0 && prob_a[1] > 0 && (form < 5 || (prob_b[0] > 0 && prob_b[1] > 0)), "debug_gemm_plan: empty problem");
  for (int i = 0; i < 26; ++i) out[i] = -1;
  int slot = 0;
  auto at = [&](bool off) { return (float*)(uintptr_t)(0x10000000ul * ++slot + (off ? 4 : 0)); };
  static const int live_blocks = 0;
  auto problem = [&](const int64_t* d) {
    GemmArgs g = gemm_stored((int)d[3], (int)d[4], at(d[12] & 1), d[5], at(d[12] & 2), d[6], at(false), d[7], (int)d[0], (int)d[1], (int)d[2]);
    g.batch_z1((int)d[8], d[0] * d[2], d[1] * d[2], d[0] * d[1]).batch_z2((int)d[9], d[8] * d[0] * d[2], d[8] * d[1] * d[2], d[8] * d[0] * d[1]);
    float* ws = at(d[12] & 4);
    if (d[11] > 0) g.split_ws(ws, d[11]);
    if (d[10]) g.rb = g.rb_n = &live_blocks, g.rb_mode = (int)d[10];
    return g;
  };
  auto show = [&](const GemmArgs& g, const GemmPlan& p, int32_t* o) {
    o[0] = p.ok;
    if (!p.ok) return;
    o[1] = p.interior, o[2] = p.splits, o[3] = p.ksplit, o[4] = p.widen, o[5] = p.rb_mode, o[6] = g.vecA, o[7] = g.vecB, o[8] = (int32_t)p.tiles;
    o[9] = p.reduce, o[10] = p.zero_fill, o[11] = p.grid;
  };
  if (form < 5) {
    GemmArgs g = problem(prob_a);
    show(g, gemm_plan(g, (GemmForm)form, splits, group_work, cap), out);
    return 0;
  }
  const DynPairForm& f = form == 5 ? pair_wx : form == 6 ? pair_ww : pair_xx;
  const GemmArgs in[2] = {problem(prob_a), problem(prob_b)};
  GemmArgs g[2] = {in[0], in[1]};
  DynPairPlan pp = dyn_pair_plan(f, g, cap);
  for (int i = 0; i < 2; ++i) {
    if (!pp.fused) g[i] = in[i], pp.p[i] = gemm_plan(g[i], f.dyn[i] == 1 ? GEMM_DYN_M : GEMM_DYN_K, 1, 0, cap);
    show(g[i], pp.p[i], out + 12 * i);
  }
  out[24] = pp.fused, out[25] = pp.fused ? pp.gridW : -1;
  return 0;
}

}
```

gcgcn_amd/csrc/gemm.hpp:

```cpp
#pragma once
#include "common.hpp"

namespace gc {

struct GemmArgs {
  const float* A = nullptr;
  const float* B = nullptr;
  float* C = nullptr;
  int M = 0, N = 0, K = 0;
  long lda = 0, ldb = 0, ldc = 0;
  int a_kc = 1, b_kc = 0;
  int batch1 = 1, batch2 = 1;
  long sA1 = 0, sA2 = 0, sB1 = 0, sB2 = 0, sC1 = 0, sC2 = 0;
  float alpha = 1.f;
  const float* add = nullptr;
  long ldadd = 0, sAdd1 = 0, sAdd2 = 0;
  const float* bias = nullptr;
  const float* rowadd = nullptr;
  long sRa1 = 0, sRa2 = 0;
  const float* rowscale = nullptr;
  long sRs1 = 0, sRs2 = 0;
  int relu = 0;
  int accumulate = 0;
  float* C2 = nullptr;
// ... 22 lines not shown

__host__ __device__ inline GemmArgs gemm_stored(int a_kc, int b_kc, const float* A, long lda, const float* B, long ldb, float* C, long ldc,
                                                int M, int N, int K) {
  GemmArgs g;
  g.A = A, g.lda = lda, g.a_kc = a_kc;
  g.B = B, g.ldb = ldb, g.b_kc = b_kc;
  g.C = C, g.ldc = ldc;
  g.M = M, g.N = N, g.K = K;
  return g;
}
__host__ __device__ inline GemmArgs gemm_nn(const float* A, long lda, const float* B, long ldb, float* C, long ldc, int M, int N, int K) {
  return gemm_stored(1, 0, A, lda, B, ldb, C, ldc, M, N, K);
}
__host__ __device__ inline GemmArgs gemm_nt(const float* A, long lda, const float* B, long ldb, float* C, long ldc, int M, int N, int K) {
  return gemm_stored(1, 1, A, lda, B, ldb, C, ldc, M, N, K);
}
__host__ __device__ inline GemmArgs gemm_tn(const float* A, long lda, const float* B, long ldb, float* C, long ldc, int M, int N, int K) {
  return gemm_stored(0, 0, A, lda, B, ldb, C, ldc, M, N, K);
}

int gemm(const GemmArgs& g, hipStream_t stream, int tile = 0, int splits = 0);

constexpr int COL_RIDE_SLICES = 64;
struct ColRide {
  const float* X = nullptr;
  float* out = nullptr;
  float* part = nullptr;
  long R = 0, ld = 0;
  int C = 0;
  int ready_slices = 0;
  ColRide stage2(int slices) const {
    ColRide c = *this;
    c.ready_slices = slices;
    return c;
  }
};
inline ColRide col_sum(const float* X, long R, long ld, int C, float* out, float* part) {
  ColRide c;
  c.X = X, c.out = out, c.part = part, c.R = R, c.ld = ld, c.C = C;
  return c;
}
inline ColRide head_sum(const float* W, int H, int D, float* out) {
  ColRide c;
  c.X = W, c.out = out, c.R = H, c.ld = D, c.C = D * D, c.ready_slices = -1;
  return c;
}
int col_sum_stage2_launch(const ColRide& c, hipStream_t stream);

template <int NP>
struct GemmGroupT {
  static constexpr int MAXP = NP;
  GemmArgs p[NP];
  int tile_begin[NP + 1];
  int tile_count[NP];
  int tile_first[NP];
  int tile_take[NP];
  int red_begin[NP + 1];
  int nprob;
  ColRide col;
};
struct MhaPass {
  const float* Q = nullptr;
  const float* P = nullptr;
  const float* dA = nullptr;
  float* dQ = nullptr;
  int N = 0, D = 0, H = 0, dh = 0, kchunk = 0, count = 0;
  float alpha = 1.f;
  Drop drop = {nullptr, 0, 0, 1.f};
};
using GemmGroup = GemmGroupT<9>;
using GemmGroup4 = GemmGroupT<4>;
int gemm_group(const GemmArgs* probs, int n, hipStream_t stream, const ColRide* col = nullptr, bool* col_later = nullptr,
               const MhaPass* mha = nullptr);
int gemm_group_mha_chunk(int dh);

struct DeferQueue {
  static constexpr int CAP = 32;
  GemmArgs p[CAP];
  int done[CAP] = {};
  int n = 0;
  static constexpr int COLCAP = 4;
  ColRide col2[COLCAP];
  int ncol2 = 0;
};
bool gemm_defer(DeferQueue* q, const GemmArgs& g);
bool gemm_defer_col2(DeferQueue* q, const ColRide& c);
bool gemm_take_deferred_col2(DeferQueue* q, ColRide& out);
int gemm_take_deferred(DeferQueue* q, GemmGroup& gg, double* flops);
int gemm_take_deferred_pairs(DeferQueue* q, GemmGroup4& gg, double* flops, long max_wgs, bool small_first = false);
int gemm_flush_deferred(DeferQueue* q, hipStream_t stream);

int splitk_reduce(const GemmArgs& g, hipStream_t st, const char* what = "gemm_splitk_reduce");

int gemm_dyn(const GemmArgs& g, const int* cnt, int dyn, long cap, hipStream_t st);
int gemm_dyn_pair(const GemmArgs& gw, const GemmArgs& gx, const int* cnt, long cap, hipStream_t st);
int gemm_dyn_pair_ww(const GemmArgs& ga, const GemmArgs& gb, const int* cnt, long cap, hipStream_t st);
int gemm_dyn_pair_xx(const GemmArgs& ga, const GemmArgs& gb, const int* cnt, long cap, hipStream_t st);

inline long gemm_ws_elems(long rows, long cols) {
  long need = 16 * rows * cols;
  const long cap = 16L << 20;
  return need < cap ? need : cap;
}

}
```

gcgcn_amd/csrc/gemm_body.hpp:

```cpp
#pragma once
#include "gemm.hpp"
#include <type_traits>

namespace gc {

typedef float f32x16 __attribute__((ext_vector_type(16)));

constexpr int BK = 32;
#ifndef GC_GEMM_EG
#define GC_GEMM_EG 4
#endif
#ifndef GC_GEMM_PF
#define GC_GEMM_PF 2
#endif

template <int BMN, bool KC, bool ALIGNED>
__device__ __forceinline__ void load_tile(float (&r)[BMN / 32][4], const float* __restrict__ src, long ld, int mn0, int k0,
                                          int MN, int Kend, int vec, int t) {
#pragma unroll
  for (int q = 0; q < BMN / 32; ++q) {
    const int f = t + 256 * q;
    int row, col, rlim, clim;
    if (KC) {
      row = mn0 + (f >> 3);
// ... 560 lines not shown
      for (int u = 0; u < 16; ++u) s += (q0 + u < cr.ready_slices) ? v[u] : 0.f;
    }
    cr.out[c] = s;
  }
}

__device__ __forceinline__ int xcd_remap(int b, int nwg) {
  const int xcd = b & 7, q = nwg >> 3, r = nwg & 7;
  return (xcd < r ? xcd * (q + 1) : r * (q + 1) + (xcd - r) * q) + (b >> 3);
}

__device__ __forceinline__ void tile_of(int q, const int count, const int tn, const int tm, int& bx, int& by, int& zs) {
  q = xcd_remap(q, count);
  zs = q / (tn * tm);
  const int r = q - zs * (tn * tm);
  bx = (tm < tn) ? r / tm : r % tn, by = (tm < tn) ? r % tm : r / tn;
}
__device__ __forceinline__ bool tile_of_rows(const GemmArgs& g, const int q, const int tn, const int tm, int& bx, int& by, int& zs,
                                             int& wide) {
  const int nl = __builtin_amdgcn_readfirstlane(*g.rb_n);
  const int tml = min((nl + 3) >> 2, tm);
  wide = split_width(g, tml, tm);
  const int live = tml * tn * g.splits * wide;
  if (q < live) {
    tile_of(q, live, tn, tml, bx, by, zs);
    return true;
  }
  if (!g.rb_zero || g.splits > 1) return false;
  const int d = q - live;
  by = tml + d / tn, bx = d - (d / tn) * tn, zs = 0;
  return by < tm;
}

template <bool RB = false, class G>
__device__ __forceinline__ void gemm_group_block(const G& gg, int hb, float* __restrict__ lds) {
  int i = 0;
  while (i + 1 < gg.nprob && hb >= gg.tile_begin[i + 1]) ++i;
  int b = hb - gg.tile_begin[i];
  if (b >= gg.tile_take[i]) return;
  const GemmArgs& g = gg.p[i];
  const int tn = g.N >> 6, tm = g.M >> 6;
  int bx, by, zs, wide = 1;
  if (RB && g.rb && g.rb_mode == 1) {
    if (!tile_of_rows(g, b + gg.tile_first[i], tn, tm, bx, by, zs, wide)) return;
  } else {
    tile_of(b + gg.tile_first[i], gg.tile_count[i], tn, tm, bx, by, zs);
  }
  const int t = threadIdx.x;
  const PlainOperands po;
  if (g.a_kc) {
    if (g.b_kc) gemm_body<1, 1, true, true, true, GC_GEMM_EG, 0, EPI_ALL, PlainOperands, RB>(g, lds, bx, by, zs, t, true, po, nullptr, 0, wide);
    else gemm_body<1, 1, true, false, true, GC_GEMM_EG, 0, EPI_ALL, PlainOperands, RB>(g, lds, bx, by, zs, t, true, po, nullptr, 0, wide);
  } else {
    if (g.b_kc) gemm_body<1, 1, false, true, true, GC_GEMM_EG, 0, EPI_ALL, PlainOperands, RB>(g, lds, bx, by, zs, t, true, po, nullptr, 0, wide);
    else gemm_body<1, 1, false, false, true, GC_GEMM_EG, 0, EPI_ALL, PlainOperands, RB>(g, lds, bx, by, zs, t, true, po, nullptr, 0, wide);
  }
}

template <class G>
__device__ __forceinline__ void gemm_group_splitk_block(const G& gg, int hb, float* __restrict__ lds, int team_lds,
                                                        float* __restrict__ xchg) {
  int i = 0;
  while (i + 1 < gg.nprob && hb >= gg.tile_begin[i + 1]) ++i;
  int q = hb - gg.tile_begin[i];
  if (q >= gg.tile_take[i]) return;
  q = xcd_remap(q + gg.tile_first[i], gg.tile_count[i]);
  const int team = threadIdx.x >> 8, t = threadIdx.x & 255;
  GemmArgs g = gg.p[i];
  const int tn = g.N >> 6, tm = g.M >> 6;
  const int z = q / (tn * tm), r = q - z * (tn * tm);
  const int bx = (tm < tn) ? r / tm : r % tn, by = (tm < tn) ? r % tm : r / tn;
  g.splits = 2, g.ksplit = g.K >> 1;
  float* tl = lds + team * team_lds;
  const int zs = z * 2 + team, role = team ? 1 : 2;
  if (g.a_kc) {
    if (g.b_kc) gemm_body<1, 1, true, true, true>(g, tl, bx, by, zs, t, true, PlainOperands(), xchg, role);
    else gemm_body<1, 1, true, false, true>(g, tl, bx, by, zs, t, true, PlainOperands(), xchg, role);
  } else {
    if (g.b_kc) gemm_body<1, 1, false, true, true>(g, tl, bx, by, zs, t, true, PlainOperands(), xchg, role);
    else gemm_body<1, 1, false, false, true>(g, tl, bx, by, zs, t, true, PlainOperands(), xchg, role);
  }
}

template <int TM, int TN, bool AKC, bool BKC>
constexpr int lds_floats() {
  return (((2 * BK * (AKC ? 64 * TM + 1 : 64 * TM)) + 3) & ~3) + 2 * BK * (BKC ? 64 * TN + 1 : 64 * TN);
}

}
```

gcgcn_amd/csrc/rowops.hip:

```cpp
#include "gat_body.hpp"
#include "gemm.hpp"
#include "rowops.hpp"

namespace gc {

constexpr int RW = 4;

__global__ __launch_bounds__(64 * RW) void softmax_fwd_kernel(const float* __restrict__ S, const float* __restrict__ coladd,
                                                              const int* __restrict__ n_valid, float* __restrict__ P,
                                                              float* __restrict__ A, long rows, int N, int heads,
                                                              Drop drop) {
  const long r = (long)blockIdx.x * RW + (threadIdx.x >> 6);
  if (r >= rows) return;
  const int lane = threadIdx.x & 63;
  const long doc = r / ((long)heads * N);
  const int i = (int)(r % N);
  const int nv = n_valid ? min(max(n_valid[doc], 0), N) : N;
  const float* s = S + r * N;
  float* p = P + r * N;
  float* a = A ? A + r * N : nullptr;
  if (i >= nv) {
    for (int j = lane; j < N; j += 64) {
      p[j] = 0.f;
      if (a) a[j] = 0.f;
    }
    return;
  }
  const float* ca = coladd ? coladd + doc * N : nullptr;
  float m = -INFINITY;
  for (int j = lane; j < nv; j += 64) m = fmaxf(m, s[j] + (ca ? ca[j] : 0.f));
  m = wave_max(m);
  float sum = 0.f;
  for (int j = lane; j < nv; j += 64) sum += expf(s[j] + (ca ? ca[j] : 0.f) - m);
  sum = wave_sum(sum);
  const float inv = 1.f / sum;
  const bool dd = a && drop.snap;
  const uint64_t key = dd ? drop_key(drop) : 0;
  for (int j = lane; j < N; j += 64) {
    float v = 0.f;
    if (j < nv) v = expf(s[j] + (ca ? ca[j] : 0.f) - m) * inv;
    p[j] = v;
    if (a) {
      if (dd) v = (rng_u32(key, (uint64_t)(r * N + j)) >= drop.thresh) ? v * drop.scale : 0.f;
      a[j] = v;
    }
  }
}

__global__ __launch_bounds__(64 * RW) void softmax_bwd_kernel(const float* __restrict__ P, const float* __restrict__ dA,
                                                              float* __restrict__ dS, long rows, int N, Drop drop) {
  const long r = (long)blockIdx.x * RW + (threadIdx.x >> 6);
  if (r >= rows) return;
  const int lane = threadIdx.x & 63;
  const float* p = P + r * N;
  const float* da = dA + r * N;
  float* ds = dS + r * N;
  const bool dd = drop.snap != nullptr;
  const uint64_t key = dd ? drop_key(drop) : 0;
  float dot = 0.f;
  for (int j = lane; j < N; j += 64) {
    float g = da[j];
    if (dd) g = (rng_u32(key, (uint64_t)(r * N + j)) >= drop.thresh) ? g * drop.scale : 0.f;
    dot = fmaf(g, p[j], dot);
  }
  dot = wave_sum(dot);
  for (int j = lane; j < N; j += 64) {
    float g = da[j];
    if (dd) g = (rng_u32(key, (uint64_t)(r * N + j)) >= drop.thresh) ? g * drop.scale : 0.f;
    ds[j] = p[j] * (g - dot);
  }
}

__global__ __launch_bounds__(64 * RW) void rowsum_inv_kernel(const float* __restrict__ A, float* __restrict__ rinv,
                                                             long rows, int N) {
  const long r = (long)blockIdx.x * RW + (threadIdx.x >> 6);
  if (r >= rows) return;
  const int lane = threadIdx.x & 63;
  float s = 0.f;
  for (int j = lane; j < N; j += 64) s += A[r * N + j];
  s = wave_sum(s);
  if (lane == 0) rinv[r] = 1.f / (s + (s == 0.f ? 1.f : 0.f));
}

__global__ __launch_bounds__(64 * RW) void relu_norm_bwd_kernel(const float* __restrict__ dY, const float* __restrict__ Y,
// ... 70 lines not shown
    return;
  }
  const long e = (long)blockIdx.x * 256 + threadIdx.x;
  if (e >= M * D) return;
  const long m = e / D;
  const int c = (int)(e - m * D);
  float s = 0.f;
  for (int h = 0; h < H; ++h) {
    const long o = (m * H + h) * D + c;
    const float g = dHO[o];
    s += g;
    if (dd) dY[o] = (rng_u32(key, (uint64_t)o) >= drop.thresh) ? g * drop.scale : 0.f;
    else if (dY != dHO) dY[o] = g;
  }
  dXres[e] = s;
}

__global__ __launch_bounds__(256) void dropout_kernel(const float* __restrict__ x, float* __restrict__ y, long n, Drop drop) {
  const long e = (long)blockIdx.x * 256 + threadIdx.x;
  if (e >= n) return;
  const uint64_t key = drop_key(drop);
  y[e] = (rng_u32(key, (uint64_t)e) >= drop.thresh) ? x[e] * drop.scale : 0.f;
}

__global__ void dropout_keep_kernel(unsigned char* keep, long n, Drop drop) {
  const long e = (long)blockIdx.x * 256 + threadIdx.x;
  if (e >= n) return;
  keep[e] = rng_u32(drop_key(drop), (uint64_t)e) >= drop.thresh;
}

__global__ void rng_next_kernel(uint64_t* state, uint64_t* snaps, int count) {
  const uint64_t seed = state[0], ctr = state[1];
  for (int i = threadIdx.x; i < count; i += 64) {
    snaps[2 * i] = seed;
    snaps[2 * i + 1] = ctr + (uint64_t)i;
  }
  __syncthreads();
  if (threadIdx.x == 0) state[1] = ctr + (uint64_t)count;
}

__global__ __launch_bounds__(256) void colsum_kernel(const float* __restrict__ X, const float* __restrict__ w,
                                                     float* __restrict__ out, long R, int C, long ld, long sXz, long sWz,
                                                     long sOz, long rows_per_split, int accumulate) {
  __shared__ float red[4][64];
  const int lane = threadIdx.x & 63, wave = threadIdx.x >> 6;
  const int c = blockIdx.x * 64 + lane;
  const int sp = blockIdx.y, z = blockIdx.z;
  const long r0 = sp * rows_per_split;
  long r1 = r0 + rows_per_split;
  if (r1 > R) r1 = R;
  const float* x = X + z * sXz;
  const float* ww = w ? w + z * sWz : nullptr;
  float acc = 0.f;
  if (c < C) {
    long r = r0 + wave;
    for (; r + 28 < r1; r += 32) {
      float v[8], wv[8];
#pragma unroll
      for (int u = 0; u < 8; ++u) v[u] = x[(r + 4 * u) * ld + c], wv[u] = ww ? ww[r + 4 * u] : 1.f;
#pragma unroll
      for (int u = 0; u < 8; ++u) acc = fmaf(wv[u], v[u], acc);
    }
    for (; r < r1; r += 4) acc = fmaf(ww ? ww[r] : 1.f, x[r * ld + c], acc);
  }
  red[wave][lane] = acc;
  __syncthreads();
  if (wave == 0 && c < C) {
    const float s = red[0][lane] + red[1][lane] + red[2][lane] + red[3][lane];
    float* o = out + z * sOz + (long)sp * C + c;
    *o = accumulate ? *o + s : s;
  }
}

struct ColJobs {
  static constexpr int MAXJ = 4;
  const float* X[MAXJ];
  const float* w[MAXJ];
  float* out[MAXJ];
  long R[MAXJ], ld[MAXJ];
  int C[MAXJ];
  long part_off[MAXJ];
  int n;
};
__global__ __launch_bounds__(256) void colsum_multi_kernel(const ColJobs j, float* __restrict__ scratch, int ns, int stage) {
  __shared__ float red[4][64];
  const int job = blockIdx.z;
  const int lane = threadIdx.x & 63, wave = threadIdx.x >> 6;
  const int C = j.C[job];
  const int c = blockIdx.x * 64 + lane;
  if (blockIdx.x * 64 >= C) return;
  float acc = 0.f;
  if (stage == 0) {
    const long R = j.R[job], rps = (R + ns - 1) / ns;
    const long r0 = (long)blockIdx.y * rps;
    const long r1 = r0 + rps < R ? r0 + rps : R;
    const float* x = j.X[job];
    const float* w = j.w[job];
    const long ld = j.ld[job];
    if (c < C) {
      long r = r0 + wave;
      for (; r + 28 < r1; r += 32) {
        float v[8], wv[8];
#pragma unroll
        for (int u = 0; u < 8; ++u) v[u] = x[(r + 4 * u) * ld + c], wv[u] = w ? w[r + 4 * u] : 1.f;
#pragma unroll
        for (int u = 0; u < 8; ++u) acc = fmaf(wv[u], v[u], acc);
      }
      for (; r < r1; r += 4) acc = fmaf(w ? w[r] : 1.f, x[r * ld + c], acc);
    }
  } else {
    const float* x = scratch + j.part_off[job];
    if (c < C) {
      int r = wave;
      for (; r + 28 < ns; r += 32) {
        float v[8];
#pragma unroll
        for (int u = 0; u < 8; ++u) v[u] = x[(long)(r + 4 * u) * C + c];
#pragma unroll
        for (int u = 0; u < 8; ++u) acc += v[u];
      }
      for (; r < ns; r += 4) acc += x[(long)r * C + c];
    }
  }
  red[wave][lane] = acc;
  __syncthreads();
  if (wave == 0 && c < C) {
    const float s = red[0][lane] + red[1][lane] + red[2][lane] + red[3][lane];
    if (stage == 0) scratch[j.part_off[job] + (long)blockIdx.y * C + c] = s;
    else j.out[job][c] = s;
  }
}

constexpr int FW = 16;
constexpr int FC = 16;
__global__ __launch_bounds__(64 * FW) void gat_fold_fwd_kernel(const float* __restrict__ flat, float* __restrict__ uvc, int D,
                                                               int Dh, uint64_t* rng_state, uint64_t* rng_snaps,
                                                               int rng_count) {
  __shared__ float red[2][64][FC + 1];
  __shared__ float redc[FW];
  if (rng_state && blockIdx.x == 0 && threadIdx.x < 64) {
    const uint64_t seed = rng_state[0], ctr = rng_state[1];
    for (int i = threadIdx.x; i < rng_count; i += 64) rng_snaps[2 * i] = seed, rng_snaps[2 * i + 1] = ctr + (uint64_t)i;
    if (threadIdx.x == 0) rng_state[1] = ctr + (uint64_t)rng_count;
  }
  const long DD = (long)Dh * D;
  const float* Wh = flat;
  const float* bh = Wh + DD;
  const float* Wt = bh + Dh;
  const float* bt = Wt + DD;
  const float* Wr = bt + Dh;
  const float* br = Wr + DD;
  const float* wt = br + Dh;
  const int lane = threadIdx.x & 63, wave = threadIdx.x >> 6;
  const int cl = threadIdx.x & (FC - 1), rl = threadIdx.x >> 4;
  const int k = blockIdx.x * FC + cl;
  float au = 0.f, av = 0.f;
  if (k < D) {
#pragma unroll 4
    for (int d = rl; d < Dh; d += 64) {
      au = fmaf(Wh[(long)d * D + k], wt[d], au);
      au = fmaf(Wt[(long)d * D + k], wt[Dh + d], au);
      av = fmaf(Wr[(long)d * D + k], wt[2 * Dh + d], av);
    }
  }
  red[0][rl][cl] = au;
  red[1][rl][cl] = av;
  __syncthreads();
  if (threadIdx.x < 2 * FC) {
    const int which = threadIdx.x / FC, c = threadIdx.x - which * FC, kk = blockIdx.x * FC + c;
    if (kk < D) {
      float sacc = 0.f;
#pragma unroll 8
      for (int r = 0; r < 64; ++r) sacc += red[which][r][c];
      uvc[which * D + kk] = sacc;
    }
  }
  if (blockIdx.x == 0) {
    float c = 0.f;
    for (int d = threadIdx.x; d < Dh; d += 64 * FW) c += wt[d] * bh[d] + wt[Dh + d] * bt[d] + wt[2 * Dh + d] * br[d];
    c = wave_sum(c);
    if (lane == 0) redc[wave] = c;
    __syncthreads();
    if (threadIdx.x == 0) {
      float tot = wt[3 * Dh];
      for (int w = 0; w < FW; ++w) tot += redc[w];
      uvc[2 * D] = tot;
    }
  }
}

__global__ __launch_bounds__(64 * FW) void gat_fold_bwd_kernel(const float* __restrict__ flat, const float* __restrict__ duvc,
                                                               float* __restrict__ dflat, int D, int Dh,
                                                               const float* __restrict__ part, long off_dv, long off_dc,
                                                               int ns) {
  extern __shared__ float sduvc[];
  if (ns > 0) {
    for (int k = threadIdx.x; k < 2 * D + 1; k += 64 * FW) {
      const float* src = k < D ? part + k : (k < 2 * D ? part + off_dv + (k - D) : part + off_dc);
      const int C = k < 2 * D ? D : 1;
      float a = 0.f;
      int q = 0;
      for (; q + 16 <= ns; q += 16) {
        float v[16];
#pragma unroll
        for (int u = 0; u < 16; ++u) v[u] = src[(long)(q + u) * C];
#pragma unroll
        for (int u = 0; u < 16; ++u) a += v[u];
      }
      for (; q < ns; ++q) a += src[(long)q * C];
      sduvc[k] = a;
    }
    __syncthreads();
    duvc = sduvc;
  }
// ... 154 lines not shown
}
int softmax_bwd(const float* P, const float* dA, float* dS, long rows, int N, Drop drop, hipStream_t st) {
  if (rows == 0) return 0;
  ProfScope ps("softmax_bwd", st);
  hipLaunchKernelGGL(softmax_bwd_kernel, dim3(cdiv(rows, RW)), dim3(64 * RW), 0, st, P, dA, dS, rows, N, drop);
  return check_launch("softmax_bwd");
}
int rowsum_inv(const float* A, float* rinv, long rows, int N, hipStream_t st) {
  if (rows == 0) return 0;
  ProfScope ps("rowsum_inv", st);
  hipLaunchKernelGGL(rowsum_inv_kernel, dim3(cdiv(rows, RW)), dim3(64 * RW), 0, st, A, rinv, rows, N);
  return check_launch("rowsum_inv");
}
int relu_norm_bwd(const float* dY, const float* Y, const float* rinv, float* dM, float* drow, long rows_m, int N, int H,
                  int L, int gh, int l, int first, hipStream_t st, int relu) {
  ProfScope ps("relu_norm_bwd", st);
  hipLaunchKernelGGL(relu_norm_bwd_kernel, dim3(cdiv(rows_m * H, RW)), dim3(64 * RW), 0, st, dY, Y, rinv, dM, drow,
                     rows_m, N, H, L, gh, l, first, relu);
  return check_launch("relu_norm_bwd");
}
int head_sum_drop_bwd(const float* dHO, float* dY, float* dXres, long M, int H, int D, Drop drop, hipStream_t st,
                      const ColRide* finish) {
  ProfScope ps("head_sum_drop_bwd", st);
  const int vec = D % 4 == 0 && ((((uintptr_t)dHO) | ((uintptr_t)dY) | ((uintptr_t)dXres)) & 15) == 0;
  const int main_blocks = cdiv(vec ? M * D / 4 : M * D, 256), extra = finish ? cdiv(finish->C, 256) : 0;
  hipLaunchKernelGGL(head_sum_drop_bwd_kernel, dim3(main_blocks + extra), dim3(256), 0, st, dHO, dY, dXres, M, H, D, drop,
                     main_blocks, finish ? finish->part : nullptr, finish ? finish->out : nullptr, finish ? finish->C : 0, vec);
  return check_launch("head_sum_drop_bwd");
}
int dropout(const float* x, float* y, long n, Drop drop, hipStream_t st) {
  GC_REQUIRE(drop.snap, "dropout: no rng snapshot");
  if (n == 0) return 0;
  ProfScope ps("dropout", st);
  hipLaunchKernelGGL(dropout_kernel, dim3(cdiv(n, 256)), dim3(256), 0, st, x, y, n, drop);
  return check_launch("dropout");
}
int dropout_keep(unsigned char* keep, long n, Drop drop, hipStream_t st) {
  GC_REQUIRE(drop.snap, "dropout_keep: no rng snapshot");
  if (n == 0) return 0;
  hipLaunchKernelGGL(dropout_keep_kernel, dim3(cdiv(n, 256)), dim3(256), 0, st, keep, n, drop);
  return check_launch("dropout_keep");
}
int rng_next(void* state, void* snaps, int count, hipStream_t st) {
  hipLaunchKernelGGL(rng_next_kernel, dim3(1), dim3(64), 0, st, (uint64_t*)state, (uint64_t*)snaps, count);
  return check_launch("rng_next");
}

constexpr int COLSUM_MIN_ROWS = 32;
constexpr int COLSUM_MAX_SPLITS = 128;
long colsum_scratch_elems(long R, int C, int batch) {
  if (R < 2 * COLSUM_MIN_ROWS) return 0;
  long ns = R / COLSUM_MIN_ROWS;
  if (ns > COLSUM_MAX_SPLITS) ns = COLSUM_MAX_SPLITS;
  return ns * C * batch;
}
int colsum(const float* X, const float* w, float* out, long R, int C, long ld, int batch, long sXz, long sWz, long sOz,
           int accumulate, float* scratch, hipStream_t st) {
  if (C == 0 || batch == 0) return 0;
  long ns = 1;
  if (R >= 2 * COLSUM_MIN_ROWS && scratch) {
    ns = R / COLSUM_MIN_ROWS;
    if (ns > COLSUM_MAX_SPLITS) ns = COLSUM_MAX_SPLITS;
    const long want = 512 / ((long)cdiv(C, 64) * batch) + 1;
    if (ns > want) ns = want;
    if (ns < 2) ns = 1;
  }
  ProfScope ps("colsum", st);
  if (ns == 1) {
    hipLaunchKernelGGL(colsum_kernel, dim3(cdiv(C, 64), 1, batch), dim3(256), 0, st, X, w, out, R, C, ld, sXz, sWz, sOz,
                       R > 0 ? R : 1, accumulate);
    return check_launch("colsum");
  }
  const long rps = (R + ns - 1) / ns;
  hipLaunchKernelGGL(colsum_kernel, dim3(cdiv(C, 64), (unsigned)ns, batch), dim3(256), 0, st, X, w, scratch, R, C, ld, sXz,
                     sWz, ns * C, rps, 0);
  if (int e = check_launch("colsum/1")) return e;
  hipLaunchKernelGGL(colsum_kernel, dim3(cdiv(C, 64), 1, batch), dim3(256), 0, st, scratch, (const float*)nullptr, out, ns, C,
                     (long)C, ns * C, 0L, sOz, ns, accumulate);
  return check_launch("colsum/2");
}

int colsum3(const float* X0, const float* w0, float* o0, long R0, int C0, long ld0, const float* X1, const float* w1,
            float* o1, long R1, int C1, long ld1, const float* X2, const float* w2, float* o2, long R2, int C2, long ld2,
            float* scratch, hipStream_t st, bool stage2, long* part_off, int* ns_out) {
  ColJobs j;
  j.n = 3;
  const float* Xs[3] = {X0, X1, X2};
  const float* ws[3] = {w0, w1, w2};
  float* os[3] = {o0, o1, o2};
  const long Rs[3] = {R0, R1, R2}, lds[3] = {ld0, ld1, ld2};
  const int Cs[3] = {C0, C1, C2};
  const int ns = stage2 ? 64 : 32;
  long off = 0;
  int maxC = 1;
  for (int i = 0; i < 3; ++i) {
    j.X[i] = Xs[i], j.w[i] = ws[i], j.out[i] = os[i], j.R[i] = Rs[i], j.ld[i] = lds[i], j.C[i] = Cs[i];
    j.part_off[i] = off;
    if (part_off) part_off[i] = off;
    off += (long)ns * Cs[i];
    if (Cs[i] > maxC) maxC = Cs[i];
  }
  if (ns_out) *ns_out = ns;
  {
    ProfScope ps("colsum", st);
    hipLaunchKernelGGL(colsum_multi_kernel, dim3(cdiv(maxC, 64), ns, 3), dim3(256), 0, st, j, scratch, ns, 0);
  }
  if (int e = check_launch("colsum3/1")) return e;
  if (!stage2) return 0;
  ProfScope ps("colsum", st);
  hipLaunchKernelGGL(colsum_multi_kernel, dim3(cdiv(maxC, 64), 1, 3), dim3(256), 0, st, j, scratch, ns, 1);
  return check_launch("colsum3/2");
}

int gat_fold_fwd(const float* flat, float* uvc, int D, int Dh, hipStream_t st, void* rng_state, void* rng_snaps,
                 int rng_count) {
  ProfScope ps("gat_fold_fwd", st);
  hipLaunchKernelGGL(gat_fold_fwd_kernel, dim3(cdiv(D, FC)), dim3(64 * FW), 0, st, flat, uvc, D, Dh, (uint64_t*)rng_state,
                     (uint64_t*)rng_snaps, rng_count);
  return check_launch("gat_fold_fwd");
}
int gat_fold_bwd(const float* flat, const float* duvc, float* dflat, int D, int Dh, hipStream_t st, const float* part,
                 const long* part_off, int ns) {
  ProfScope ps("gat_fold_bwd", st);
  const size_t lds = ns > 0 ? sizeof(float) * (2 * (size_t)D + 1) : 0;
  hipLaunchKernelGGL(gat_fold_bwd_kernel, dim3(cdiv(Dh, FW)), dim3(64 * FW), lds, st, flat, duvc, dflat, D, Dh, part,
                     ns > 0 ? part_off[1] : 0L, ns > 0 ? part_off[2] : 0L, ns);
  return check_launch("gat_fold_bwd");
}
int gat_dlogit_slices(int D) { return D >= 256 ? 8 : (D >= 64 ? 4 : 1); }
int gat_dlogit(const float* P, const float* dA, const float* uvc, const float* dXin, float* dlogit, float* ds, float* dX,
               int B, int N, int D, int slices, Drop drop, hipStream_t st) {
  GC_REQUIRE(N <= GT && slices > 0, "gat_dlogit: N=%d slices=%d", N, slices);
  ProfScope ps("gat_dlogit", st);
  hipLaunchKernelGGL(gat_dlogit_kernel, dim3(B, slices), dim3(256), 0, st, P, dA, uvc, dXin, dlogit, ds, dX, N, D, drop);
  return check_launch("gat_dlogit");
}
int node_score_fwd(const float* X, const float* uvc, float* s, long M, int D, hipStream_t st, void* rng_state, void* rng_snaps,
                   int rng_count) {
  ProfScope ps("node_score_fwd", st);
  hipLaunchKernelGGL(node_score_fwd_kernel, dim3(cdiv(M, RW)), dim3(64 * RW), 0, st, X, uvc, s, M, D, (uint64_t*)rng_state,
                     (uint64_t*)rng_snaps, rng_count);
  return check_launch("node_score_fwd");
}
int node_score_bwd(const float* ds, const float* uvc, const float* dXin, float* dX, long M, int D, hipStream_t st) {
  ProfScope ps("node_score_bwd", st);
  hipLaunchKernelGGL(node_score_bwd_kernel, dim3(cdiv(M * D, 256)), dim3(256), 0, st, ds, uvc, dXin, dX, M, D);
  return check_launch("node_score_bwd");
}
int mask_rows(const float* x, float* y, long M, int D, int N, const int* n_valid, Drop drop, hipStream_t st, const float* wlin,
              float* wsum, int H) {
  ProfScope ps("mask_rows", st);
  const int vec = x && D % 4 == 0 && ((((uintptr_t)x) | ((uintptr_t)y)) & 15) == 0;
  const int main_blocks = x ? cdiv(vec ? M * D / 4 : M * D, 256) : 0, extra = wsum ? cdiv((long)D * D, 256) : 0;
  if (main_blocks + extra == 0) return 0;
  hipLaunchKernelGGL(mask_rows_kernel, dim3(main_blocks + extra), dim3(256), 0, st, x, y, M, D, N, n_valid, drop, main_blocks,
                     wlin, wsum, H, vec);
  return check_launch("mask_rows");
}

}
```

gcgcn_amd/csrc/rowops.hpp:

```cpp
#pragma once
#include "common.hpp"

namespace gc {

int softmax_fwd(const float* S, const float* coladd, const int* n_valid, float* P, float* A, long rows, int N, int heads,
                Drop drop, hipStream_t st);
int softmax_bwd(const float* P, const float* dA, float* dS, long rows, int N, Drop drop, hipStream_t st);
int rowsum_inv(const float* A, float* rinv, long rows, int N, hipStream_t st);
int relu_norm_bwd(const float* dY, const float* Y, const float* rinv, float* dM, float* drow, long rows_m, int N, int H,
                  int L, int gh, int l, int first, hipStream_t st, int relu = 1);
struct ColRide;
struct DeferQueue;
int head_sum_drop_bwd(const float* dHO, float* dY, float* dXres, long M, int H, int D, Drop drop, hipStream_t st,
                      const ColRide* finish = nullptr);
int dropout(const float* x, float* y, long n, Drop drop, hipStream_t st);
int dropout_keep(unsigned char* keep, long n, Drop drop, hipStream_t st);
int rng_next(void* state, void* snaps, int count, hipStream_t st);
long colsum_scratch_elems(long R, int C, int batch);
int colsum(const float* X, const float* w, float* out, long R, int C, long ld, int batch, long sXz, long sWz, long sOz,
           int accumulate, float* scratch, hipStream_t st);
int colsum3(const float* X0, const float* w0, float* o0, long R0, int C0, long ld0, const float* X1, const float* w1,
            float* o1, long R1, int C1, long ld1, const float* X2, const float* w2, float* o2, long R2, int C2, long ld2,
            float* scratch, hipStream_t st, bool stage2 = true, long* part_off = nullptr, int* ns_out = nullptr);
int gat_fold_fwd(const float* flat, float* uvc, int D, int Dh, hipStream_t st, void* rng_state = nullptr,
                 void* rng_snaps = nullptr, int rng_count = 0);
int gat_fold_bwd(const float* flat, const float* duvc, float* dflat, int D, int Dh, hipStream_t st,
                 const float* part = nullptr, const long* part_off = nullptr, int ns = 0);
int gat_dlogit_slices(int D);
struct GatTail;
int gat_dlogit(const float* P, const float* dA, const float* uvc, const float* dXin, float* dlogit, float* ds, float* dX,
               int B, int N, int D, int slices, Drop drop, hipStream_t st);
int node_score_fwd(const float* X, const float* uvc, float* s, long M, int D, hipStream_t st, void* rng_state = nullptr,
                   void* rng_snaps = nullptr, int rng_count = 0);
int node_score_bwd(const float* ds, const float* uvc, const float* dXin, float* dX, long M, int D, hipStream_t st);
int mask_rows(const float* x, float* y, long M, int D, int N, const int* n_valid, Drop drop, hipStream_t st,
              const float* wlin = nullptr, float* wsum = nullptr, int H = 0);

int edge_fwd(const float* E, const float* v, const int* n_valid, float* Ebar, const float* coladd, float* P, float* A,
             Drop drop, int B, int N, int D, hipStream_t st, const unsigned char* mask = nullptr);
struct EdgePlan;
int edge_bwd(const float* E, const float* v, const int* n_valid, const float* dlogit, const float* dEbar, float* dE,
             float* dvpart, const EdgePlan& plan, int B, int N, int D, hipStream_t st, DeferQueue* carry = nullptr,
             const GatTail* tail = nullptr);
int edge_bcast(const float* dEbar, const int* n_valid, float* dE, int B, int N, int D, hipStream_t st);

int row_blocks(const int* n_valid, int B, int N, int* out, hipStream_t st);
constexpr int ROWBLK_HDR = 4;
constexpr int ROWBLK_LIST_MAX = 512;
static inline long row_blocks_ints(int B, int N) { return ROWBLK_HDR + (long)B * N / 16; }

int pair_bce_fwd(const float* logits, const float* labels, const int* n_valid, float* loss, float* part, int B, int N, int R,
                 hipStream_t st);
int pair_bce_bwd(const float* logits, const float* labels, const int* n_valid, const float* dloss, float* dlogits, int B, int N,
                 int R, hipStream_t st);

int64_t eval_ws_bytes(int64_t n_records, int64_t n_keep);
int eval_scan(const float* logits, const float* labels, const uint8_t* in_train, const int* n_valid, const int64_t* doc_base,
              uint64_t* rec, int64_t capacity, int64_t* counters, int B, int N, int R, hipStream_t st);
int eval_rank(const uint64_t* rec, int64_t n, void* ws, int64_t ws_bytes, int64_t* sorted_off, hipStream_t st);
int eval_curve(const uint64_t* keys, int64_t m, const int64_t* counters, double input_theta, float* pr_x, float* pr_y,
               float* ign_pr_y, double* res, void* ws, int64_t ws_bytes, int64_t n_records, hipStream_t st);

}
```

gcgcn_amd/functional.py:

```python
from __future__ import annotations

import ctypes
import os
import threading
import weakref
from typing import Optional

import torch
from torch.autograd.function import once_differentiable

from . import _lib
from ._lib import SALT_GLUE, call

Tensor = torch.Tensor


def _p(t: Optional[Tensor]):
    return None if t is None else t.data_ptr()


_raw_stream = getattr(torch._C, "_cuda_getCurrentRawStream", None)


def _stream():
# ... 85 lines not shown
        return False


def _take_pending_rng(dev: torch.device):
    sc = _get_scope()
    if sc is not None and sc[2] and sc[0].device == dev:
        sc[2] = False
        return _state(dev), sc[0], sc[0].shape[0]
    return None


def rng_snapshot(dev: torch.device, lazy: bool = False) -> Tensor:
    sc = _get_scope()
    if sc is not None and sc[1] < sc[0].shape[0] and sc[0].device == dev:
        if sc[2] and not lazy:
            sc[2] = False
            call("gcgcn_rng_next", _p(_state(dev)), _p(sc[0]), sc[0].shape[0], _stream())
        snap = sc[0][sc[1]]
        sc[1] += 1
        return snap
    return _new_snaps(dev, 1)[0]


def dropout_keep_mask(snap: Tensor, salt: int, p: float, numel: int) -> Tensor:
    keep = torch.empty(numel, dtype=torch.uint8, device=snap.device)
    call("gcgcn_dropout_keep", _p(keep), numel, _p(snap), salt, float(p), _stream())
    return keep.bool()


def _gat_fwd_buffers(x: Tensor, snap, pending, uvc, uvc_valid):
    B, N, D = x.shape
    dev = x.device
    rng = pending if pending is not None else (None, None, 0)
    if uvc is None:
        uvc, uvc_valid = torch.empty(2 * D + 1, device=dev), False
    s = torch.empty(B, N, device=dev)
    P = torch.empty(B, N, N, device=dev)
    A = torch.empty(B, N, N, device=dev) if snap is not None else None
    ebar = torch.empty(B, N, D, device=dev)
    return uvc, uvc_valid, s, P, A, ebar, rng


def _gat_bwd_buffers(x: Tensor, dA, dEbar, dXin, scratch_elems: str):
    B, N, D = x.shape
    dev = x.device
    dA = torch.zeros(B, N, N, device=dev) if dA is None else dA.contiguous()
    dEbar = None if dEbar is None else dEbar.contiguous()
    dXin = None if dXin is None else dXin.contiguous()
    dlogit = torch.empty(B, N, N, device=dev)
    ds = torch.empty(B, N, device=dev)
    dvpart = torch.empty(B * N, D, device=dev)
    duvc = torch.empty(2 * D + 1, device=dev)
    scratch = torch.empty(max(getattr(_lib.lib(), scratch_elems)(B, N, D), 1), device=dev)
    return dA, dEbar, dXin, dlogit, ds, dvpart, duvc, scratch


class GatFn(torch.autograd.Function):

    @staticmethod
    def forward(ctx, x, e, flat, n_valid, p, snap, pending, Dh, mask, uvc, uvc_valid):
        B, N, D = x.shape
        uvc, uvc_valid, s, P, A, ebar, (st, sn, cnt) = _gat_fwd_buffers(x, snap, pending, uvc, uvc_valid)
        call("gcgcn_gat_fwd", B, N, D, Dh, _p(x), _p(e), _p(n_valid), _p(flat), _p(snap), float(p), _p(uvc), _p(s),
             _p(P), _p(A), _p(ebar), _p(st), _p(sn), cnt, _p(mask), 1 if uvc_valid else 0, _stream())
        ctx.save_for_backward(x, e, flat, uvc, P)
        ctx.n_valid, ctx.p, ctx.snap, ctx.Dh, ctx.mask = n_valid, float(p), snap, Dh, mask
        return (P if A is None else A), ebar, x.view_as(x)

    @staticmethod
    def backward(ctx, dA, dEbar, dXin):
        x, e, flat, uvc, P = ctx.saved_tensors
        B, N, D = x.shape
        dev = x.device
        dA, dEbar, dXin, dlogit, ds, dvpart, duvc, scratch = _gat_bwd_buffers(x, dA, dEbar, dXin, "gcgcn_gat_bwd_scratch")
        if ctx.mask is not None:
            gone = ctx.mask.bool()
            if ctx.n_valid is not None:
                gone = gone | (torch.arange(N, device=dev)[None, None, :] >= ctx.n_valid[:, None, None])
            dA = dA.masked_fill(gone.all(-1, keepdim=True), 0.0)
        dX = torch.empty_like(x)
        dE = torch.empty_like(e) if ctx.needs_input_grad[1] else None
        dflat = torch.empty_like(flat)
        bp = _current_pass()
        call("gcgcn_gat_bwd", B, N, D, ctx.Dh, _p(x), _p(e), _p(ctx.n_valid), _p(flat), _p(ctx.snap), ctx.p, _p(uvc), _p(P),
             _p(dA), _p(dEbar), _p(dXin), _p(dX), _p(dE), _p(dflat), _p(dlogit), _p(ds), _p(dvpart), _p(duvc),
             _p(scratch), None if bp is None else bp.queue, _stream())
        return dX, dE, dflat, None, None, None, None, None, None, None, None


class EdgeMeanFn(torch.autograd.Function):

    @staticmethod
    def forward(ctx, e, n_valid):
        B, N, _, D = e.shape
        ebar = torch.empty(B, N, D, device=e.device)
        call("gcgcn_edge_mean_fwd", B, N, D, _p(e), _p(n_valid), _p(ebar), _stream())
        ctx.n_valid, ctx.shape = n_valid, (B, N, D)
        return ebar

    @staticmethod
    def backward(ctx, dEbar):
        B, N, D = ctx.shape
        dEbar = dEbar.contiguous()
        dE = torch.empty(B, N, N, D, device=dEbar.device)
        call("gcgcn_edge_mean_bwd", B, N, D, _p(dEbar), _p(ctx.n_valid), _p(dE), _stream())
        return dE, None


class MhaFn(torch.autograd.Function):

    @staticmethod
    def forward(ctx, x, flat, n_valid, H, p, snap, rowblk=None):
        B, N, D = x.shape
        dev = x.device
        Q = torch.empty(B, N, D, device=dev)
        P = torch.empty(B, H, N, N, device=dev)
        A = torch.empty(B, H, N, N, device=dev) if snap is not None else None
        scratch = torch.empty(max(_lib.lib().gcgcn_mha_scratch(B, N, D), 1), device=dev)
        call("gcgcn_mha_fwd", B, N, D, H, _p(x), _p(n_valid), _p(flat), _p(snap), float(p), _p(Q), _p(P), _p(A),
             _p(scratch), _p(rowblk), _stream())
        ctx.save_for_backward(x, flat, Q, P)
        ctx.H, ctx.p, ctx.snap, ctx.rowblk = H, float(p), snap, rowblk
        return (P if A is None else A), x.view_as(x)

    @staticmethod
    def backward(ctx, dA, dXin):
        x, flat, Q, P = ctx.saved_tensors
        B, N, D = x.shape
        H, dev = ctx.H, x.device
        dA = torch.zeros(B, H, N, N, device=dev) if dA is None else dA.contiguous()
        dXin = None if dXin is None else dXin.contiguous()
        dX = torch.empty_like(x)
        dflat = torch.empty_like(flat)
        dS = torch.empty(B, H, N, N, device=dev)
        dQ = torch.empty(B, N, D, device=dev)
        scratch = torch.empty(max(_lib.lib().gcgcn_mha_scratch(B, N, D), 1), device=dev)
        call("gcgcn_mha_bwd", B, N, D, H, _p(x), _p(flat), _p(ctx.snap), ctx.p, _p(Q), _p(P), _p(dA), _p(dXin), _p(dX),
             _p(dflat), _p(dS), _p(dQ), _p(scratch), None, 0, _p(ctx.rowblk), _stream())
        return dX, dflat, None, None, None, None, None


defer_weight_grads = os.environ.get("GCGCN_DEFER", "1") != "0"
defer_fused_mha_weight_grads = os.environ.get("GCGCN_DEFER_MHA", "1") != "0"
_warned_ddp = [False]


def _under_ddp() -> bool:
    ddp = getattr(torch.nn.parallel, "DistributedDataParallel", None)
    if ddp is not None and not hasattr(ddp, "_active_ddp_module"):
        import torch.distributed as dist
        on = dist.is_available() and dist.is_initialized() and dist.get_world_size() > 1
    else:
        on = ddp is not None and getattr(ddp, "_active_ddp_module", None) is not None
    if on and defer_weight_grads and not _warned_ddp[0]:
        _warned_ddp[0] = True
        import warnings
        warnings.warn("gcgcn_amd: running under torch DistributedDataParallel -- deferred weight gradients are switched off "
                      "for these blocks (their AccumulateGrad hooks need the gradient during backward); "
                      "gcgcn_amd.dist.FlatGradBucket reduces the flat gradients without that cost")
    return on
_passes = {}
_passes_lock = threading.Lock()


class _BackwardPass:
    def __init__(self, task_id: int):
        self.task_id = task_id
        self.queue = _lib.lib().gcgcn_defer_create()
        if not self.queue:
            raise MemoryError("gcgcn_defer_create failed")
        self.keep = []
        self.installs = []

    def park(self, leaf, dflat, operands):
        self.keep.append(operands)
        self.installs.append((leaf, dflat))

    def __call__(self):
        with _passes_lock:
            _passes.pop(self.task_id, None)
        try:
            if _lib.lib().gcgcn_defer_count(self.queue) > 0:
                call("gcgcn_defer_flush", self.queue, _stream())
            with torch.no_grad():
                for leaf, dflat in self.installs:
                    if leaf.grad is None:
                        leaf.grad = dflat
                    else:
                        leaf.grad.add_(dflat)
        finally:
            self.keep.clear()
            self.installs.clear()

    def __del__(self):
        q, self.queue = self.queue, None
        if q:
            try:
                _lib.lib().gcgcn_defer_destroy(q)
            except Exception:
                pass


def _current_pass() -> Optional[_BackwardPass]:
    tid = torch._C._current_graph_task_id()
    if tid < 0:
        return None
    ref = _passes.get(tid)
    return None if ref is None else ref()


def _pass_for_parking(ctx, idx: int, leaf=None) -> Optional[_BackwardPass]:
    if not (defer_weight_grads and ctx.needs_input_grad[idx]):
        return None
    leaf = ctx.flat_leaf if leaf is None else leaf
    if leaf is None or leaf._post_accumulate_grad_hooks or leaf._backward_hooks:
        return None
    tid = torch._C._current_graph_task_id()
    if tid < 0:
        return None
    try:
        acc = ctx.next_functions[idx][0]
        if acc is None or getattr(acc, "variable", None) is not leaf or torch._C._will_engine_execute_node(acc) is not True:
            return None
    except RuntimeError:
        return None
    with _passes_lock:
        ref = _passes.get(tid)
        bp = None if ref is None else ref()
        if bp is None:
            bp = _BackwardPass(tid)
            _passes[tid] = weakref.ref(bp)
            torch.autograd.Variable._execution_engine.queue_callback(bp)
            for k in [k for k, r in _passes.items() if r() is None]:
                del _passes[k]
    return bp


def _ride(inp, n_valid, out, B, N, D):
    r = _lib.EdgeRide(B, N, D, inp.data_ptr(), None if n_valid is None else n_valid.data_ptr(), out.data_ptr())
    return r, ctypes.cast(ctypes.pointer(r), ctypes.c_void_p)


head_sum_in_forward = True


def _gcn_forward(ctx, x, ebar, adj, flat, n_valid, L, H, p, snap, e_next, out_p, out_snap, rowblk, hook=None, saved=()):
    B, N, D = x.shape
    dev = x.device
    HD = H * D
    out = torch.empty(B, N, D, device=dev)
    Pn, Y, HO = (torch.empty(B, N, HD, device=dev) for _ in range(3))
    if hook is None:
        rinv = torch.empty(B, H, N, device=dev)
        G = torch.empty(B, N, HD, device=dev)
    else:
        G = torch.empty(B, N, HD, device=dev)
        rinv = torch.empty(B, H, N, device=dev)
    wsum = torch.empty(D, D, device=dev) if (H > 1 and head_sum_in_forward and any(ctx.needs_input_grad[:4])) else None
    scratch = torch.empty(max(_lib.lib().gcgcn_gcn_scratch(B, N, D, H), 1), device=dev)
# ... 735 lines not shown
```

include/gcgcn.h:

```cpp
#ifndef GCGCN_H
#define GCGCN_H
#include <stdint.h>

#ifdef __cplusplus
extern "C" {
#endif

int gcgcn_version(void);
const char* gcgcn_last_error(void);

int gcgcn_set_option(const char* name, int value);

int64_t gcgcn_row_blocks_ints(int B, int N);
int gcgcn_row_blocks(int B, int N, const int32_t* n_valid, int32_t* out, void* stream);

int gcgcn_prof_start(const char* kernel_prefix, int capacity);
int gcgcn_prof_enable(int on);
int gcgcn_prof_stop(double* total_ms, int* launches, double* work);

int gcgcn_rng_next(void* state, void* snaps, int count, void* stream);
int gcgcn_dropout_keep(uint8_t* keep, int64_t n, const void* rng_snap, uint64_t salt, float p, void* stream);
int gcgcn_dropout(const float* x, float* y, int64_t n, const void* rng_snap, uint64_t salt, float p, void* stream);

#define GCGCN_SALT_GAT 0x47415431ull
#define GCGCN_SALT_MHA 0x4d484131ull
#define GCGCN_SALT_GCN 0x47434e31ull
#define GCGCN_SALT_GLUE 0x474c5531ull

int gcgcn_gat_layout(int D, int Dh, int64_t* out9);

int gcgcn_gat_fwd(int B, int N, int D, int Dh, const float* X, const float* E, const int32_t* n_valid, const float* flat,
                  const void* rng_snap, float p, float* uvc, float* s, float* P, float* A, float* Ebar, void* rng_state,
                  void* rng_snaps, int rng_count, const uint8_t* mask, int uvc_valid, void* stream);

int64_t gcgcn_gat_bwd_scratch(int B, int N, int D);
int gcgcn_gat_bwd(int B, int N, int D, int Dh, const float* X, const float* E, const int32_t* n_valid, const float* flat,
                  const void* rng_snap, float p, const float* uvc, const float* P, const float* dA, const float* dEbar,
                  const float* dX_in, float* dX, float* dE, float* dflat, float* dlogit, float* ds, float* dvpart,
                  float* duvc, float* scratch, void* defer_queue, void* stream);

int gcgcn_edge_mean_fwd(int B, int N, int D, const float* E, const int32_t* n_valid, float* Ebar, void* stream);
int gcgcn_edge_mean_bwd(int B, int N, int D, const float* dEbar, const int32_t* n_valid, float* dE, void* stream);

int gcgcn_mha_layout(int D, int64_t* out3);
int64_t gcgcn_mha_scratch(int B, int N, int D);
int gcgcn_mha_fwd(int B, int N, int D, int H, const float* X, const int32_t* n_valid, const float* flat,
                  const void* rng_snap, float p, float* Q, float* P, float* A, float* scratch, const int32_t* rowblk, void* stream);
int gcgcn_mha_bwd(int B, int N, int D, int H, const float* X, const float* flat, const void* rng_snap, float p,
                  const float* Q, const float* P, const float* dA, const float* dX_in, float* dX, float* dflat,
                  float* dS, float* dQ, float* scratch, void* defer_queue, int core_done, const int32_t* rowblk, void* stream);

int gcgcn_gcn_layout(int D, int L, int H, int64_t* out7);
int64_t gcgcn_gcn_scratch(int B, int N, int D, int H);
typedef struct gcgcn_edge_ride {
  int32_t B, N, D;
  const float* in;
  const int32_t* n_valid;
  float* out;
} gcgcn_edge_ride;
typedef struct gcgcn_mha_hook {
  const float* flat_q;
  float* Q;
  float* P;
  float* A;
  float* dQ;
  const void* rng_snap;
  float p;
} gcgcn_mha_hook;
int gcgcn_maggc_fusable(int N, int D, int H);
int gcgcn_gcn_fwd(int B, int N, int D, int L, int H, const float* X, const float* Ebar, const float* A,
                  const int32_t* n_valid, const float* flat, const void* rng_snap, float p, const void* out_rng_snap,
                  float out_p, float* out, float* Pn, float* Y, float* HO, float* rinv, float* G, float* wsum, float* scratch,
                  const gcgcn_edge_ride* ride, const gcgcn_mha_hook* mha, const int32_t* rowblk, void* stream);
int gcgcn_gcn_bwd(int B, int N, int D, int L, int H, const float* X, const float* Ebar, const float* A,
                  const int32_t* n_valid, const float* flat, const void* rng_snap, float p, const void* out_rng_snap,
                  float out_p, const float* Pn, const float* Y, const float* HO, const float* rinv, const float* wsum,
                  const float* dout, float* dX, float* dEbar,
                  float* dA, float* dflat, float* W1, float* W2, float* W3, float* drow, float* dXres, float* dout_m,
                  float* scratch, const gcgcn_edge_ride* ride, const gcgcn_mha_hook* mha, void* defer_queue, const int32_t* rowblk,
                  void* stream);
void* gcgcn_defer_create(void);
void gcgcn_defer_destroy(void* queue);
int gcgcn_defer_count(const void* queue);
int gcgcn_defer_flush(void* queue, void* stream);

int gcgcn_graphconv_fwd(int B, int N, int Din, int De, int Dout, const float* X, const float* Ebar, const float* A,
                        const float* We, const float* Wn, const float* bias, float* out, float* T, float* rinv,
                        float* scratch, void* stream);
int gcgcn_graphconv_bwd(int B, int N, int Din, int De, int Dout, const float* X, const float* Ebar, const float* A,
                        const float* We, const float* Wn, const float* out, const float* T, const float* rinv,
                        const float* dout, float* dX, float* dEbar, float* dA, float* dWe, float* dWn, float* dbias,
                        float* dS, float* dT, float* drow, float* scratch, void* stream);

int gcgcn_pair_bce_fwd(int B, int N, int R, const float* logits, const float* labels, const int32_t* n_valid, float* loss,
                       float* part, void* stream);
int gcgcn_pair_bce_bwd(int B, int N, int R, const float* logits, const float* labels, const int32_t* n_valid,
                       const float* dloss, float* dlogits, void* stream);

int64_t gcgcn_eval_ws_bytes(int64_t n_records, int64_t n_keep);
int gcgcn_eval_scan(int B, int N, int R, const float* logits, const float* labels, const uint8_t* in_train, const int32_t* n_valid,
                    const int64_t* doc_base, uint64_t* records, int64_t capacity, int64_t* counters, void* stream);
int gcgcn_eval_rank(const uint64_t* records, int64_t n, void* ws, int64_t ws_bytes, int64_t* sorted_off, void* stream);
int gcgcn_eval_curve(const uint64_t* ranked, int64_t m, int64_t n_records, const int64_t* counters, double input_theta,
                     float* pr_x, float* pr_y, float* ign_pr_y, double* result, void* ws, int64_t ws_bytes, void* stream);

int gcgcn_producer_layout(int Hd, int P, int64_t* out17);
int gcgcn_producer_count(int B, int N, int S, int T, const uint8_t* sen, const int32_t* n_valid, int32_t* counts2, void* stream);
int gcgcn_producer_sizes(int B, int N, int S, int T, int Hd, int P, int ND, int64_t cap_rows, int64_t cap_pairs, int64_t* out7);
int gcgcn_producer_fwd(int B, int N, int S, int T, int Hd, int P, int ND, const float* ctx, const uint8_t* sen, const void* pos_h,
                       const void* pos_t, int pos_bytes, const float* node, const float* dis_table, const int32_t* n_valid,
                       const float* flat, int64_t cap_rows, int64_t cap_pairs, int32_t* ibuf, float* fbuf, float* scratch,
                       int64_t scratch_elems, float* E, void* stream);
int gcgcn_producer_bwd(int B, int N, int S, int T, int Hd, int P, int ND, const float* ctx, const uint8_t* sen, const void* pos_h,
                       const void* pos_t, int pos_bytes, const float* node, const float* dis_table, const int32_t* n_valid,
                       const float* flat, int64_t cap_rows, int64_t cap_pairs, int32_t* ibuf, float* fbuf, float* bbuf,
                       const float* dE, const float* dEc, float* dctx, float* dnode, float* ddis_table, float* dflat, void* stream);

int gcgcn_edge_mean_fwd_compact(int B, int N, int D, const float* Ec, const int32_t* prow, const float* bias, const int32_t* n_valid,
                                float* Ebar, void* stream);
int gcgcn_edge_mean_bwd_compact(int B, int N, int D, const int32_t* prow, const int32_t* n_valid, const float* dEbar, float* dEc,
                                float* dbias, float* rowbuf, void* stream);
int gcgcn_gat_fwd_compact(int B, int N, int D, int Dh, const float* X, const float* Ec, const int32_t* prow, const float* bias,
                          const int32_t* n_valid, const float* flat, const void* rng_snap, float p, float* uvc, float* s, float* P,
                          float* A, float* Ebar, void* rng_state, void* rng_snaps, int rng_count, int uvc_valid, void* stream);
int64_t gcgcn_gat_bwd_compact_scratch(int B, int N, int D);
int gcgcn_gat_bwd_compact(int B, int N, int D, int Dh, const float* X, const float* Ec, const int32_t* prow, const float* bias,
                          const int32_t* n_valid, const float* flat, const void* rng_snap, float p, const float* uvc, const float* P,
                          const float* dA, const float* dEbar, const float* dX_in, float* dX, float* dEc, float* dbias, float* dflat,
                          float* dlogit, float* ds, float* dvpart, float* duvc, float* scratch, void* stream);

int gcgcn_head_layout(int Hd, int nf, int Pt, int Pr, int R, int64_t* out7);
int gcgcn_head_sizes(int B, int N, int R, int ND, int64_t* out3);
int gcgcn_head_fwd(int B, int N, int Hd, int nf, int Pt, int Pr, int R, int ND, int dis_plus, const float* const* feats,
                   const int64_t* node_type, const int64_t* node_relative_pos, const float* ner_emb, const float* dis_table,
                   const int32_t* n_valid, const float* flat, float* fbuf, int32_t* ibuf, float* logits, void* stream);
int gcgcn_head_bwd(int B, int N, int Hd, int nf, int Pt, int Pr, int R, int ND, int dis_plus, const float* const* feats,
                   const int64_t* node_type, const int64_t* node_relative_pos, const float* ner_emb, const float* dis_table,
                   const int32_t* n_valid, const float* flat, float* fbuf, int32_t* ibuf, float* bbuf, const float* dlogits,
                   float* const* dfeats, float* dner_emb, float* ddis_table, float* dflat, void* stream);

int gcgcn_tensorise(int B, int N, int S, int T, int R, int dis_plus, int n_slots, const int32_t* slots, int n_edges,
                    const int32_t* edges, int n_labels, const int32_t* labels, int n_mentions, const int32_t* mentions,
                    const int32_t* mention_node, const int32_t* n_valid, const int32_t* first_start, float* adj, uint8_t* sen, uint8_t* pos_h,
                    uint8_t* pos_t, float* node_pos, int64_t* node_relative_pos, float* label_matrix, void* stream);

int gcgcn_debug_spread(int64_t n_tiles, int64_t n_others, int64_t cohort, int64_t pct, int32_t* kind, int32_t* ordinal);

int gcgcn_debug_chain_plan(int bwd, int B, int N, int D, int L, int H, int ragged, int ride, int hook, int scratch,
                           int misalign, int32_t* out);

int gcgcn_debug_head_plan(int B, int N, int R, int ragged, int32_t* out);

int gcgcn_debug_edge_plan(int pass, int compact, int B, int N, int D, int ragged, int att, int has_dE, int has_dEbar, int misalign,
                          int parked_tiles, int any_rb, int col_C, int32_t* out);

int gcgcn_debug_attn_plan(int bwd, int N, int D, int H, int hook, int chain_attends, int core_done, int misalign, int32_t* out);

int gcgcn_debug_out_bwd_plan(int fuse, int B, int N, int D, int H, int scratch, int wsum_fwd, int ragged, int odrop, int drop,
                             int dxres_misaligned, int front_reduced, int32_t* out);

int gcgcn_debug_gemm_plan(int form, const int64_t* prob_a, const int64_t* prob_b, int splits, int64_t group_work, int64_t cap,
                          int32_t* out);

int gcgcn_gemm(int M, int N, int K, const float* A, int64_t lda, int a_kc, const float* B, int64_t ldb, int b_kc,
               float* C, int64_t ldc, int batch, int64_t sA, int64_t sB, int64_t sC, float alpha, const float* bias,
               int relu, int accumulate, int tile, int splits, float* ws, int64_t ws_elems, void* stream);

int gcgcn_gemm_dyn(int M, int N, int K, const float* A, int64_t lda, int a_kc, const float* B, int64_t ldb, int b_kc, float* C,
                   int64_t ldc, const float* bias, int accumulate, const int32_t* count, int dyn, int64_t cap, float* ws,
                   int64_t ws_elems, void* stream);

int gcgcn_adam_step(int n_tensors, const void* table, int64_t total_blocks, double beta1, double beta2, double eps, void* stream);

int64_t gcgcn_adam_ws_bytes(int n_tensors, int64_t total_blocks);
int gcgcn_adam_step_dev(int n_tensors, const void* table, int64_t total_blocks, double beta1, double beta2, double eps,
                        const float* lr, double max_norm, void* ws, int64_t ws_bytes, float* grad_norm, void* stream);

int64_t gcgcn_lstm_ws_bytes(int B, int T, int I, int H, int nd);
int gcgcn_lstm_fwd(int B, int T, int I, int H, int nd, const float* x, const float* w_ih, const float* w_hh, const float* bias,
                   const float* h0, const float* c0, float* out, float* gates, float* csave, void* stream);
int gcgcn_lstm_bwd(int B, int T, int I, int H, int nd, const float* x, const float* w_ih, const float* w_hh, const float* h0,
                   const float* c0, const float* out, const float* gates, const float* csave, const float* dout, float* dgates,
                   float* dx, float* dw_ih, float* dw_hh, float* db, float* dh0, float* dc0, void* ws, int64_t ws_bytes, void* stream);

int64_t gcgcn_frontend_ws_bytes(int B, int T, int V, int P, int R, int Dw, int Dc, int Dn, int K);
int gcgcn_embed_fwd(int B, int T, int V, int P, int R, int Dw, int Dc, int Dn, const int64_t* document, const int64_t* document_pos,
                    const int64_t* document_ner, const float* word_w, const float* coref_w, const float* ner_w, const float* scale,
                    float* x, void* stream);
int gcgcn_embed_bwd(int B, int T, int V, int P, int R, int Dw, int Dc, int Dn, const int64_t* document, const int64_t* document_pos,
                    const int64_t* document_ner, const float* dx, const float* scale, int coref_padding_idx, int ner_padding_idx,
                    float* dword, float* dcoref, float* dner, void* ws, int64_t ws_bytes, void* stream);
int gcgcn_context_fwd(int B, int T, int N, int K, int Hd, const float* h, const float* w, const float* bias, const float* node_pos,
                      float* pre, float* ctx, float* node_feat, void* stream);
int gcgcn_context_bwd(int B, int T, int N, int K, int Hd, const float* h, const float* w, const float* node_pos, const float* ctx,
                      const float* dctx, const float* dnode_feat, float* dpre, float* dh, float* dw, float* db, void* ws,
                      int64_t ws_bytes, void* stream);

#ifdef __cplusplus
}
#endif
#endif
```

Baseline: 65970 docs/s.

## K-split GEMMs carried on the edge backward kernel and fuse their reduction into colsum

When the deferred GEMM problems riding on the edge backward kernel have too few tiles to fill the GPU, each plain problem with enough K tiles is split into K slices written to a workspace slab. This gives the carry launch more workgroups. The split-K reduction is then folded into the colsum launch as extra grid planes, so it needs no separate kernel. The cost is extra workspace allocation per backward pass, the slab round-trip through memory, and more planning logic that must stay consistent with the launch grid.

```diff
diff --git a/gcgcn_amd/_lib.py b/gcgcn_amd/_lib.py
--- a/gcgcn_amd/_lib.py
+++ b/gcgcn_amd/_lib.py
@@ -38,6 +38,8 @@
     "gcgcn_debug_head_plan": (I, [I, I, I, I, P]),
     "gcgcn_debug_gemm_plan": (I, [I, P, P, I, L, L, P]),
     "gcgcn_debug_edge_plan": (I, [I] * 13 + [P]),
+    "gcgcn_debug_carry_ksplit": (I, [I, P, L, I, L, P]),
+    "gcgcn_debug_carry_stats": (I, [P]),
     "gcgcn_debug_attn_plan": (I, [I] * 8 + [P]),
     "gcgcn_debug_out_bwd_plan": (I, [I] * 12 + [P]),
     "gcgcn_prof_start": (I, [c_char_p, I]),
@@ -67,6 +69,8 @@
     "gcgcn_defer_destroy": (None, [P]),
     "gcgcn_defer_count": (I, [P]),
     "gcgcn_defer_flush": (I, [P, P]),
+    "gcgcn_defer_split_ws": (L, [P, I, I, I]),
+    "gcgcn_defer_workspace": (I, [P, P, L]),
     "gcgcn_graphconv_fwd": (I, [I, I, I, I, I, P, P, P, P, P, P, P, P, P, P, P]),
     "gcgcn_graphconv_bwd": (I, [I, I, I, I, I, P, P, P, P, P, P, P, P, P, P, P, P, P, P, P, P, P, P, P, P]),
     "gcgcn_pair_bce_fwd": (I, [I, I, I, P, P, P, P, P, P]),
diff --git a/gcgcn_amd/csrc/api.hip b/gcgcn_amd/csrc/api.hip
--- a/gcgcn_amd/csrc/api.hip
+++ b/gcgcn_amd/csrc/api.hip
@@ -208,14 +208,15 @@
     GC_TRY(colsum(dlogit, nullptr, ds, N, N, N, B, (long)N * N, 0, N, 0, nullptr, st));
     GC_TRY(node_score_bwd(ds, uvc, dX_in, dX, M, D, st));
   }
+  SplitReduce reduce;
   if (compact)
     GC_TRY(cmp_bwd(eo.ce, v, n_valid, dlogit, dEbar, dE, dvpart, scratch + plan.rowbuf_off, dbias, plan, B, N, D, st));
   else
-    GC_TRY(edge_bwd(eo.E, v, n_valid, dlogit, dEbar, dE, dvpart, plan, B, N, D, st, dq, &tail));
+    GC_TRY(edge_bwd(eo.E, v, n_valid, dlogit, dEbar, dE, dvpart, plan, B, N, D, st, dq, &tail, &reduce));
   long part_off[3];
   int ns = 0;
   GC_TRY(colsum3(X, ds, duvc, M, D, D, dvpart, nullptr, duvc + D, M, D, D, ds, nullptr, duvc + 2 * D, M, 1, 1, scratch,
-                 st, false, part_off, &ns));
+                 st, false, part_off, &ns, &reduce));
   return gat_fold_bwd(flat, duvc, dflat, D, Dh, st, scratch, part_off, ns);
 }
 
@@ -518,6 +519,16 @@
 void gcgcn_defer_destroy(void* queue) { delete (DeferQueue*)queue; }
 int gcgcn_defer_count(const void* queue) { return queue ? ((const DeferQueue*)queue)->n + ((const DeferQueue*)queue)->ncol2 : 0; }
 int gcgcn_defer_flush(void* queue, void* stream) { return gemm_flush_deferred((DeferQueue*)queue, (hipStream_t)stream); }
+int64_t gcgcn_defer_split_ws(const void* queue, int B, int N, int D) {
+  if (!queue || B <= 0 || N <= 0 || D <= 0) return 0;
+  const EdgePlan p = edge_plan_bwd({B, N, D, false, true, true, true, 0});
+  return p.carry_ok ? gemm_deferred_split_ws((const DeferQueue*)queue, p.grid) : 0;
+}
+int gcgcn_defer_workspace(void* queue, float* ws, int64_t elems) {
+  GC_REQUIRE(queue && elems >= 0 && (ws || elems == 0) && (((uintptr_t)ws) & 15) == 0, "defer_workspace: bad arguments");
+  ((DeferQueue*)queue)->ws = ws, ((DeferQueue*)queue)->ws_elems = elems;
+  return 0;
+}
 
 int gcgcn_pair_bce_fwd(int B, int N, int R, const float* logits, const float* labels, const int32_t* n_valid, float* loss,
                        float* part, void* stream) {
@@ -890,6 +901,26 @@
   return 0;
 }
 
+int gcgcn_debug_carry_ksplit(int n, const int32_t* probs, int64_t rows, int col_C, int64_t ws_have, int64_t* out) {
+  GC_REQUIRE(n >= 0 && n <= CarrySplit::MAXP && (probs || n == 0) && rows >= 0 && col_C >= 0 && ws_have >= 0 && out, "debug_carry_ksplit: bad arguments");
+  CarryProb pr[CarrySplit::MAXP];
+  for (int i = 0; i < n; ++i) {
+    GC_REQUIRE(probs[3 * i] > 0 && probs[3 * i + 1] > 0 && probs[3 * i] < (1 << 24), "debug_carry_ksplit: empty problem");
+    pr[i].tiles = probs[3 * i], pr[i].ktiles = probs[3 * i + 1], pr[i].plain = probs[3 * i + 2] != 0;
+  }
+  const CarrySplit c = edge_plan_ksplit(pr, n, rows, col_C, ws_have);
+  out[0] = c.nsplit, out[1] = c.ws_elems, out[2] = c.ntile, out[3] = c.unsplit_tiles, out[4] = c.nred, out[5] = c.grid;
+  for (int i = 0; i < CarrySplit::MAXP; ++i) out[6 + i] = i < n ? c.slices[i] : -1, out[6 + CarrySplit::MAXP + i] = i < n ? c.ws_off[i] : -1;
+  return 0;
+}
+int gcgcn_debug_carry_stats(int64_t* out) {
+  GC_REQUIRE(out, "debug_carry_stats: null pointer");
+  long v[5];
+  edge_carry_stats(v);
+  for (int i = 0; i < 5; ++i) out[i] = v[i];
+  return 0;
+}
+
 static const int64_t kEvalMaxRecords = 0xffffffffLL;
 
 int64_t gcgcn_eval_ws_bytes(int64_t n_records, int64_t n_keep) {
diff --git a/gcgcn_amd/csrc/edge.hip b/gcgcn_amd/csrc/edge.hip
--- a/gcgcn_amd/csrc/edge.hip
+++ b/gcgcn_amd/csrc/edge.hip
@@ -1,4 +1,6 @@
 #include <string.h>
+
+#include <atomic>
 
 #include "edge_body.hpp"
 #include "compact.hpp"
@@ -184,6 +186,7 @@
 }
 constexpr size_t EDGE_LDS_MAX = 160 * 1024;
 constexpr size_t CMP_LDS_MAX = 64 * 1024;
+constexpr int CARRY_SPREAD_MIN = 1024;
 constexpr size_t TILE_LDS = sizeof(float) * lds_floats<1, 1, true, true>();
 static_assert(sizeof(float) * GAT_DOC_LDS <= TILE_LDS, "GAT passenger needs more LDS than a tile");
 
@@ -231,19 +234,52 @@
   return edge_plan_bwd(m);
 }
 
-void edge_plan_carry(EdgePlan& p, int ntile, bool any_rb, int col_C) {
+void edge_plan_carry(EdgePlan& p, int ntile, bool any_rb, int col_C, int order_tiles) {
   if (ntile <= 0) return;
   const long rows = p.grid;
   p.ntile = ntile, p.RB = any_rb;
   p.ncolwg = col_C > 0 ? cdiv(col_C, 256) : 0;
   p.col_base = col_C > 0 ? (int)(rows + ntile) : 0;
   p.grid = rows + ntile + p.ncolwg;
-  constexpr int spread_pct = 90, cohort = 256, spread_min = 1024;
-  p.spread = make_spread(ntile, rows, cohort, ntile >= spread_min ? spread_pct : 0);
+  constexpr int spread_pct = 90, cohort = 256;
+  p.spread = make_spread(ntile, rows, cohort, (order_tiles < 0 ? ntile : order_tiles) >= CARRY_SPREAD_MIN ? spread_pct : 0);
   p.lds = 0;
 }
 
+CarrySplit edge_plan_ksplit(const CarryProb* pr, int n, long rows, int col_C, long ws_have) {
+  const int ksplit = option("carry_ksplit", 2), min_ktiles = option("carry_ksplit_min", 16);
+  CarrySplit c;
+  c.ws_elems = 0, c.nsplit = 0, c.unsplit_tiles = 0, c.ntile = 0, c.nred = 0;
+  for (int i = 0; i < CarrySplit::MAXP; ++i) c.slices[i] = 1, c.ws_off[i] = -1;
+  if (n > CarrySplit::MAXP) n = CarrySplit::MAXP;
+  for (int i = 0; i < n; ++i) c.unsplit_tiles = ((c.unsplit_tiles + 7) & ~7) + pr[i].tiles;
+  const bool offered = ksplit > 1 && c.unsplit_tiles < CARRY_SPREAD_MIN;
+  long need = 0;
+  for (int i = 0; i < n && offered; ++i)
+    if (pr[i].plain && pr[i].ktiles >= min_ktiles) need += (long)ksplit * pr[i].tiles * 64 * 64;
+  const bool split = offered && need > 0 && need <= ws_have;
+  for (int i = 0; i < n; ++i) {
+    if (split && pr[i].plain && pr[i].ktiles >= min_ktiles) {
+      c.slices[i] = ksplit, c.ws_off[i] = c.ws_elems;
+      c.ws_elems += (long)ksplit * pr[i].tiles * 64 * 64;
+      c.nred += pr[i].tiles * (64 * 64 / 4 / 256);
+      ++c.nsplit;
+    }
+    c.ntile = ((c.ntile + 7) & ~7) + pr[i].tiles * c.slices[i];
+  }
+  c.grid = rows + c.ntile + (col_C > 0 ? cdiv(col_C, 256) : 0);
+  return c;
+}
+
 constexpr int NT_STORE = 0;
+
+static std::atomic<long> g_carry_stats[5];
+static void carry_stats_add(const CarrySplit& cs, bool col2) {
+  g_carry_stats[0] += 1, g_carry_stats[1] += cs.nsplit, g_carry_stats[2] += cs.ntile, g_carry_stats[3] += cs.nred, g_carry_stats[4] += col2;
+}
+void edge_carry_stats(long* out) {
+  for (int i = 0; i < 5; ++i) out[i] = g_carry_stats[i].load();
+}
 
 int edge_fwd(const float* E, const float* v, const int* n_valid, float* Ebar, const float* coladd, float* P, float* A,
              Drop drop, int B, int N, int D, hipStream_t st, const unsigned char* mask) {
@@ -270,7 +306,9 @@
 }
 
 int edge_bwd(const float* E, const float* v, const int* n_valid, const float* dlogit, const float* dEbar, float* dE,
-             float* dvpart, const EdgePlan& plan, int B, int N, int D, hipStream_t st, DeferQueue* carry, const GatTail* tail) {
+             float* dvpart, const EdgePlan& plan, int B, int N, int D, hipStream_t st, DeferQueue* carry, const GatTail* tail,
+             SplitReduce* reduce) {
+  if (reduce) reduce->nprob = 0;
   GatTail gt;
   memset(&gt, 0, sizeof gt);
   if (tail && plan.route == EdgePlan::RIDE) gt = *tail;
@@ -291,7 +329,29 @@
     const bool col = gemm_take_deferred_col2(carry, gg.col);
     bool any_rb = false;
     for (int i = 0; i < gg.nprob; ++i) any_rb = any_rb || gg.p[i].rb != nullptr;
-    edge_plan_carry(p, ntile, any_rb, col ? gg.col.C : 0);
+    CarryProb pr[GemmGroup::MAXP];
+    static_assert(CarrySplit::MAXP == GemmGroup::MAXP, "CarrySplit holds one entry per carried problem");
+    const int np = gemm_carry_probs(gg, pr);
+    const CarrySplit cs = edge_plan_ksplit(pr, np, p.grid, col ? gg.col.C : 0, reduce ? carry->ws_elems : 0);
+    int launch_tiles = ntile;
+    if (cs.nsplit > 0) {
+      launch_tiles = gemm_split_carried(gg, cs, carry->ws);
+      GC_REQUIRE(launch_tiles == cs.ntile, "edge_bwd: the K-split laid out %d tile workgroups, the plan %d", launch_tiles, cs.ntile);
+      reduce->nprob = gg.nprob;
+      for (int i = 0; i < gg.nprob; ++i) reduce->p[i] = gg.p[i];
+      for (int i = 0; i <= gg.nprob; ++i) reduce->red_begin[i] = gg.red_begin[i];
+    }
+    const int order_tiles = (cs.nsplit > 0 && option("carry_ksplit_spread", 0)) ? CARRY_SPREAD_MIN : cs.unsplit_tiles;
+    edge_plan_carry(p, launch_tiles, any_rb, col ? gg.col.C : 0, order_tiles);
+    GC_REQUIRE(p.grid == cs.grid, "edge_bwd: grid %ld, the K-split plan %ld", p.grid, cs.grid);
+    carry_stats_add(cs, col);
+    if (option("group_dump", 0)) {
+      fprintf(stderr, "edge_bwd_carry: %d problems, %d tile workgroups (%d unsplit), %d reduce workgroups, slabs %ld floats, rows %ld, col2 %d\n",
+              gg.nprob, cs.ntile, cs.unsplit_tiles, cs.nred, cs.ws_elems, (long)B * N + p.ngat, col ? gg.col.C : 0);
+      for (int i = 0; i < np; ++i)
+        fprintf(stderr, "  %-12s M %5d N %5d K %5d tiles %5d k-tiles %4d plain %d slices %d\n", gg.p[i].tag, gg.p[i].M, gg.p[i].N, gg.p[i].K,
+                pr[i].tiles, pr[i].ktiles, (int)pr[i].plain, cs.slices[i]);
+    }
     dim3 grid((unsigned)p.grid);
 #define GC_EDGE_CARRY(RBV)                                                                                                  \
   GC_LAUNCH_TIMED("edge_bwd", bytes, (edge_bwd_carry_kernel<4, RBV>), grid, block, 0, st, E, v, n_valid, dlogit, dEbar, dE, \
diff --git a/gcgcn_amd/csrc/edge_plan.hpp b/gcgcn_amd/csrc/edge_plan.hpp
--- a/gcgcn_amd/csrc/edge_plan.hpp
+++ b/gcgcn_amd/csrc/edge_plan.hpp
@@ -36,6 +36,24 @@
 EdgePlan edge_plan_fwd(const EdgeQuery& q);
 EdgePlan edge_plan_bwd(const EdgeQuery& q);
 EdgePlan edge_plan_bcast(const EdgeQuery& q);
-void edge_plan_carry(EdgePlan& p, int ntile, bool any_rb, int col_C);
+void edge_plan_carry(EdgePlan& p, int ntile, bool any_rb, int col_C, int order_tiles = -1);
+
+struct CarryProb {
+  int tiles;
+  int ktiles;
+  bool plain;
+};
+struct CarrySplit {
+  static constexpr int MAXP = 9;
+  int slices[MAXP];
+  long ws_off[MAXP];
+  long ws_elems;
+  int nsplit;
+  int unsplit_tiles;
+  int ntile;
+  int nred;
+  long grid;
+};
+CarrySplit edge_plan_ksplit(const CarryProb* pr, int n, long rows, int col_C, long ws_have);
 
 }
diff --git a/gcgcn_amd/csrc/gemm.hip b/gcgcn_amd/csrc/gemm.hip
--- a/gcgcn_amd/csrc/gemm.hip
+++ b/gcgcn_amd/csrc/gemm.hip
@@ -2,6 +2,7 @@
 
 #include "attn_plan.hpp"
 #include "edge_body.hpp"
+#include "edge_plan.hpp"
 #include "gemm_body.hpp"
 #include "mha_body.hpp"
 #include "rowops.hpp"
@@ -100,67 +101,8 @@
   gemm_group_block<RB>(gg, x - before, lds);
 }
 
-__device__ __forceinline__ void reduce4(const GemmArgs& g, int z, long idx4) {
-  const long mn = (long)g.M * g.N;
-  const long idx = idx4 * 4;
-  if (idx >= mn) return;
-  const long nb = (long)g.batch1 * g.batch2;
-  int row = (int)(idx / g.N);
-  const int col = (int)(idx - (long)row * g.N);
-  const int z1 = z / g.batch2, z2 = z - z1 * g.batch2;
-  int nsplit = g.splits;
-  if (g.rb && g.rb_mode == 1) {
-    const int bi = row >> 4;
-    const int prow = g.rb[bi] * 16 + (row & 15);
-    const int tm = (g.M + 63) >> 6;
-    nsplit *= split_width(g, min((*g.rb_n + 3) >> 2, tm), tm);
-    if (bi >= *g.rb_n) {
-      if (g.rb_zero) {
-        const float4 zero = make_float4(0.f, 0.f, 0.f, 0.f);
-        float* c = g.C + z1 * g.sC1 + z2 * g.sC2 + (long)prow * g.ldc + col;
-        c[0] = 0.f, c[1] = 0.f, c[2] = 0.f, c[3] = 0.f;
-        if (g.C2) {
-          float* c2 = g.C2 + z1 * g.sC21 + z2 * g.sC22 + (long)prow * g.ldc2 + col;
-          c2[0] = zero.x, c2[1] = zero.y, c2[2] = zero.z, c2[3] = zero.w;
-        }
-      }
-      return;
-    }
-    row = prow;
-  }
-  const float4* w = reinterpret_cast<const float4*>(g.ws + (long)z * mn + idx);
-  const long stride4 = nb * mn / 4;
-  float4 acc = make_float4(0.f, 0.f, 0.f, 0.f);
-  if (nsplit <= 4) {
-    for (int s = 0; s < nsplit; ++s) {
-      const float4 v = w[(long)s * stride4];
-      acc.x += v.x, acc.y += v.y, acc.z += v.z, acc.w += v.w;
-    }
-  } else {
-    for (int s0 = 0; s0 < nsplit; s0 += 8) {
-      float4 v[8];
-#pragma unroll
-      for (int u = 0; u < 8; ++u) v[u] = w[(long)min(s0 + u, nsplit - 1) * stride4];
-#pragma unroll
-      for (int u = 0; u < 8; ++u)
-        if (s0 + u < nsplit) acc.x += v[u].x, acc.y += v[u].y, acc.z += v[u].z, acc.w += v[u].w;
-    }
-  }
-  if (!(g.add || g.bias || g.rowadd || g.rowscale || g.relu || g.accumulate || g.n_valid || g.C2) && g.alpha == 1.f) {
-    float* c = g.C + z1 * g.sC1 + z2 * g.sC2 + (long)row * g.ldc + col;
-    if ((((uintptr_t)c) & 15) == 0) {
-      *reinterpret_cast<float4*>(c) = acc;
-    } else {
-      c[0] = acc.x, c[1] = acc.y, c[2] = acc.z, c[3] = acc.w;
-    }
-    return;
-  }
-  const Epi e = make_epi(g, z1, z2);
-  epi_store4(g, e, row, col, acc);
-}
-
 __global__ __launch_bounds__(256) void splitk_reduce_group_kernel(const GemmGroup gg) {
-  int b = blockIdx.x, i = 0;
+  const int b = blockIdx.x;
   if (b >= gg.red_begin[gg.nprob]) {
     const ColRide& cr = gg.col;
     const int c = (b - gg.red_begin[gg.nprob]) * 256 + threadIdx.x;
@@ -171,13 +113,7 @@
     }
     return;
   }
-  while (i + 1 < gg.nprob && b >= gg.red_begin[i + 1]) ++i;
-  b -= gg.red_begin[i];
-  const GemmArgs& g = gg.p[i];
-  if (g.splits <= 1) return;
-  const int per = (int)(((long)g.M * g.N / 4 + 255) / 256);
-  const int z = b / per;
-  reduce4(g, z, (long)(b - z * per) * 256 + threadIdx.x);
+  splitk_reduce_group_block(gg, b);
 }
 
 __global__ __launch_bounds__(256) void splitk_reduce_kernel(const GemmArgs g) {
@@ -659,6 +595,46 @@
   return take_parked(q, gg, flops, max_wgs, small_first);
 }
 
+int gemm_carry_probs(const GemmGroup& gg, CarryProb* pr) {
+  for (int i = 0; i < gg.nprob; ++i) {
+    const GemmArgs& g = gg.p[i];
+    pr[i].tiles = gg.tile_take[i], pr[i].ktiles = cdiv(g.K, BK);
+    pr[i].plain = !g.rb && gg.tile_first[i] == 0 && gg.tile_take[i] == gg.tile_count[i] && g.splits <= 1;
+  }
+  return gg.nprob;
+}
+
+int gemm_split_carried(GemmGroup& gg, const CarrySplit& cs, float* ws) {
+  int wgs = 0, reds = 0;
+  for (int i = 0; i < gg.nprob; ++i) {
+    GemmArgs& g = gg.p[i];
+    const int s = cs.slices[i];
+    gg.red_begin[i] = reds;
+    if (s > 1) {
+      const long slab = (long)gg.tile_count[i] * 64 * 64;
+      g.splits = s, g.ksplit = cdiv(cdiv(g.K, BK), s) * BK;
+      g.split_ws(ws + cs.ws_off[i], s * slab);
+      reds += (int)(slab / 4 / 256);
+      gg.tile_count[i] *= s, gg.tile_take[i] = gg.tile_count[i];
+    }
+    wgs = (wgs + 7) & ~7;
+    gg.tile_begin[i] = wgs;
+    wgs += gg.tile_take[i];
+  }
+  gg.tile_begin[gg.nprob] = wgs, gg.red_begin[gg.nprob] = reds;
+  return wgs;
+}
+
+long gemm_deferred_split_ws(const DeferQueue* q, long rows) {
+  if (!q || q->n == 0) return 0;
+  DeferQueue c = *q;
+  GemmGroup gg;
+  if (take_parked(&c, gg, nullptr, 1L << 40) <= 0) return 0;
+  CarryProb pr[GemmGroup::MAXP];
+  const int n = gemm_carry_probs(gg, pr);
+  return edge_plan_ksplit(pr, n, rows, 0, 1L << 60).ws_elems;
+}
+
 template <bool RB>
 __global__ __launch_bounds__(256, 4) void gemm_parked_kernel(const GemmGroup gg) {
   __shared__ __attribute__((aligned(16))) float lds[lds_floats<1, 1, true, true>()];
diff --git a/gcgcn_amd/csrc/gemm.hpp b/gcgcn_amd/csrc/gemm.hpp
--- a/gcgcn_amd/csrc/gemm.hpp
+++ b/gcgcn_amd/csrc/gemm.hpp
@@ -128,11 +128,23 @@
   static constexpr int COLCAP = 4;
   ColRide col2[COLCAP];
   int ncol2 = 0;
+  float* ws = nullptr;
+  long ws_elems = 0;
+};
+struct CarryProb;
+struct CarrySplit;
+struct SplitReduce {
+  GemmArgs p[GemmGroup::MAXP];
+  int red_begin[GemmGroup::MAXP + 1];
+  int nprob = 0;
 };
 bool gemm_defer(DeferQueue* q, const GemmArgs& g);
 bool gemm_defer_col2(DeferQueue* q, const ColRide& c);
 bool gemm_take_deferred_col2(DeferQueue* q, ColRide& out);
 int gemm_take_deferred(DeferQueue* q, GemmGroup& gg, double* flops);
+int gemm_carry_probs(const GemmGroup& gg, CarryProb* pr);
+int gemm_split_carried(GemmGroup& gg, const CarrySplit& cs, float* ws);
+long gemm_deferred_split_ws(const DeferQueue* q, long rows);
 int gemm_take_deferred_pairs(DeferQueue* q, GemmGroup4& gg, double* flops, long max_wgs, bool small_first = false);
 int gemm_flush_deferred(DeferQueue* q, hipStream_t stream);
 
diff --git a/gcgcn_amd/csrc/gemm_body.hpp b/gcgcn_amd/csrc/gemm_body.hpp
--- a/gcgcn_amd/csrc/gemm_body.hpp
+++ b/gcgcn_amd/csrc/gemm_body.hpp
@@ -666,6 +666,78 @@
   }
 }
 
+__device__ __forceinline__ void reduce4(const GemmArgs& g, int z, long idx4) {
+  const long mn = (long)g.M * g.N;
+  const long idx = idx4 * 4;
+  if (idx >= mn) return;
+  const long nb = (long)g.batch1 * g.batch2;
+  int row = (int)(idx / g.N);
+  const int col = (int)(idx - (long)row * g.N);
+  const int z1 = z / g.batch2, z2 = z - z1 * g.batch2;
+  int nsplit = g.splits;
+  if (g.rb && g.rb_mode == 1) {
+    const int bi = row >> 4;
+    const int prow = g.rb[bi] * 16 + (row & 15);
+    const int tm = (g.M + 63) >> 6;
+    nsplit *= split_width(g, min((*g.rb_n + 3) >> 2, tm), tm);
+    if (bi >= *g.rb_n) {
+      if (g.rb_zero) {
+        const float4 zero = make_float4(0.f, 0.f, 0.f, 0.f);
+        float* c = g.C + z1 * g.sC1 + z2 * g.sC2 + (long)prow * g.ldc + col;
+        c[0] = 0.f, c[1] = 0.f, c[2] = 0.f, c[3] = 0.f;
+        if (g.C2) {
+          float* c2 = g.C2 + z1 * g.sC21 + z2 * g.sC22 + (long)prow * g.ldc2 + col;
+          c2[0] = zero.x, c2[1] = zero.y, c2[2] = zero.z, c2[3] = zero.w;
+        }
+      }
+      return;
+    }
+    row = prow;
+  }
+  const float4* w = reinterpret_cast<const float4*>(g.ws + (long)z * mn + idx);
+  const long stride4 = nb * mn / 4;
+  float4 acc = make_float4(0.f, 0.f, 0.f, 0.f);
+  if (nsplit <= 4) {
+    for (int s = 0; s < nsplit; ++s) {
+      const float4 v = w[(long)s * stride4];
+      acc.x += v.x, acc.y += v.y, acc.z += v.z, acc.w += v.w;
+    }
+  } else {
+    for (int s0 = 0; s0 < nsplit; s0 += 8) {
+      float4 v[8];
+#pragma unroll
+      for (int u = 0; u < 8; ++u) v[u] = w[(long)min(s0 + u, nsplit - 1) * stride4];
+#pragma unroll
+      for (int u = 0; u < 8; ++u)
+        if (s0 + u < nsplit) acc.x += v[u].x, acc.y += v[u].y, acc.z += v[u].z, acc.w += v[u].w;
+    }
+  }
+  if (!(g.add || g.bias || g.rowadd || g.rowscale || g.relu || g.accumulate || g.n_valid || g.C2) && g.alpha == 1.f) {
+    float* c = g.C + z1 * g.sC1 + z2 * g.sC2 + (long)row * g.ldc + col;
+    if ((((uintptr_t)c) & 15) == 0) {
+      *reinterpret_cast<float4*>(c) = acc;
+    } else {
+      c[0] = acc.x, c[1] = acc.y, c[2] = acc.z, c[3] = acc.w;
+    }
+    return;
+  }
+  const Epi e = make_epi(g, z1, z2);
+  epi_store4(g, e, row, col, acc);
+}
+
+template <class G>
+__device__ __forceinline__ void splitk_reduce_group_block(const G& gg, int b) {
+  if (b >= gg.red_begin[gg.nprob]) return;
+  int i = 0;
+  while (i + 1 < gg.nprob && b >= gg.red_begin[i + 1]) ++i;
+  b -= gg.red_begin[i];
+  const GemmArgs& g = gg.p[i];
+  if (g.splits <= 1) return;
+  const int per = (int)(((long)g.M * g.N / 4 + 255) / 256);
+  const int z = b / per;
+  reduce4(g, z, (long)(b - z * per) * 256 + threadIdx.x);
+}
+
 template <int TM, int TN, bool AKC, bool BKC>
 constexpr int lds_floats() {
   return (((2 * BK * (AKC ? 64 * TM + 1 : 64 * TM)) + 3) & ~3) + 2 * BK * (BKC ? 64 * TN + 1 : 64 * TN);
diff --git a/gcgcn_amd/csrc/rowops.hip b/gcgcn_amd/csrc/rowops.hip
--- a/gcgcn_amd/csrc/rowops.hip
+++ b/gcgcn_amd/csrc/rowops.hip
@@ -1,5 +1,5 @@
 #include "gat_body.hpp"
-#include "gemm.hpp"
+#include "gemm_body.hpp"
 #include "rowops.hpp"
 
 namespace gc {
@@ -236,7 +236,7 @@
   long part_off[MAXJ];
   int n;
 };
-__global__ __launch_bounds__(256) void colsum_multi_kernel(const ColJobs j, float* __restrict__ scratch, int ns, int stage) {
+__device__ __forceinline__ void colsum_multi_block(const ColJobs& j, float* __restrict__ scratch, int ns, int stage) {
   __shared__ float red[4][64];
   const int job = blockIdx.z;
   const int lane = threadIdx.x & 63, wave = threadIdx.x >> 6;
@@ -284,6 +284,16 @@
     else j.out[job][c] = s;
   }
 }
+__global__ __launch_bounds__(256) void colsum_multi_kernel(const ColJobs j, float* __restrict__ scratch, int ns, int stage) {
+  colsum_multi_block(j, scratch, ns, stage);
+}
+__global__ __launch_bounds__(256) void colsum_multi_reduce_kernel(const ColJobs j, float* __restrict__ scratch, int ns, const SplitReduce gg) {
+  if ((int)blockIdx.z >= j.n) {
+    splitk_reduce_group_block(gg, (int)(((blockIdx.z - j.n) * gridDim.y + blockIdx.y) * gridDim.x + blockIdx.x));
+    return;
+  }
+  colsum_multi_block(j, scratch, ns, 0);
+}
 
 constexpr int FW = 16;
 constexpr int FC = 16;
@@ -604,7 +614,7 @@
 
 int colsum3(const float* X0, const float* w0, float* o0, long R0, int C0, long ld0, const float* X1, const float* w1,
             float* o1, long R1, int C1, long ld1, const float* X2, const float* w2, float* o2, long R2, int C2, long ld2,
-            float* scratch, hipStream_t st, bool stage2, long* part_off, int* ns_out) {
+            float* scratch, hipStream_t st, bool stage2, long* part_off, int* ns_out, const SplitReduce* reduce) {
   ColJobs j;
   j.n = 3;
   const float* Xs[3] = {X0, X1, X2};
@@ -623,7 +633,13 @@
     if (Cs[i] > maxC) maxC = Cs[i];
   }
   if (ns_out) *ns_out = ns;
-  {
+  const int nred = (reduce && reduce->nprob > 0) ? reduce->red_begin[reduce->nprob] : 0;
+  if (nred > 0) {
+    static_assert(sizeof(ColJobs) + sizeof(SplitReduce) + 32 <= 4096, "colsum_multi_reduce_kernel: kernel arguments exceed 4 KB");
+    const int plane = cdiv(maxC, 64) * ns;
+    ProfScope ps("colsum", st);
+    hipLaunchKernelGGL(colsum_multi_reduce_kernel, dim3(cdiv(maxC, 64), ns, 3 + cdiv(nred, plane)), dim3(256), 0, st, j, scratch, ns, *reduce);
+  } else {
     ProfScope ps("colsum", st);
     hipLaunchKernelGGL(colsum_multi_kernel, dim3(cdiv(maxC, 64), ns, 3), dim3(256), 0, st, j, scratch, ns, 0);
   }
diff --git a/gcgcn_amd/csrc/rowops.hpp b/gcgcn_amd/csrc/rowops.hpp
--- a/gcgcn_amd/csrc/rowops.hpp
+++ b/gcgcn_amd/csrc/rowops.hpp
@@ -11,6 +11,7 @@
                   int L, int gh, int l, int first, hipStream_t st, int relu = 1);
 struct ColRide;
 struct DeferQueue;
+struct SplitReduce;
 int head_sum_drop_bwd(const float* dHO, float* dY, float* dXres, long M, int H, int D, Drop drop, hipStream_t st,
                       const ColRide* finish = nullptr);
 int dropout(const float* x, float* y, long n, Drop drop, hipStream_t st);
@@ -21,7 +22,8 @@
            int accumulate, float* scratch, hipStream_t st);
 int colsum3(const float* X0, const float* w0, float* o0, long R0, int C0, long ld0, const float* X1, const float* w1,
             float* o1, long R1, int C1, long ld1, const float* X2, const float* w2, float* o2, long R2, int C2, long ld2,
-            float* scratch, hipStream_t st, bool stage2 = true, long* part_off = nullptr, int* ns_out = nullptr);
+            float* scratch, hipStream_t st, bool stage2 = true, long* part_off = nullptr, int* ns_out = nullptr,
+            const SplitReduce* reduce = nullptr);
 int gat_fold_fwd(const float* flat, float* uvc, int D, int Dh, hipStream_t st, void* rng_state = nullptr,
                  void* rng_snaps = nullptr, int rng_count = 0);
 int gat_fold_bwd(const float* flat, const float* duvc, float* dflat, int D, int Dh, hipStream_t st,
@@ -41,7 +43,8 @@
 struct EdgePlan;
 int edge_bwd(const float* E, const float* v, const int* n_valid, const float* dlogit, const float* dEbar, float* dE,
              float* dvpart, const EdgePlan& plan, int B, int N, int D, hipStream_t st, DeferQueue* carry = nullptr,
-             const GatTail* tail = nullptr);
+             const GatTail* tail = nullptr, SplitReduce* reduce = nullptr);
+void edge_carry_stats(long* out);
 int edge_bcast(const float* dEbar, const int* n_valid, float* dE, int B, int N, int D, hipStream_t st);
 
 int row_blocks(const int* n_valid, int B, int N, int* out, hipStream_t st);
diff --git a/gcgcn_amd/functional.py b/gcgcn_amd/functional.py
--- a/gcgcn_amd/functional.py
+++ b/gcgcn_amd/functional.py
@@ -191,6 +191,8 @@
         dE = torch.empty_like(e) if ctx.needs_input_grad[1] else None
         dflat = torch.empty_like(flat)
         bp = _current_pass()
+        if bp is not None:
+            bp.workspace(B, N, D, dev)
         call("gcgcn_gat_bwd", B, N, D, ctx.Dh, _p(x), _p(e), _p(ctx.n_valid), _p(flat), _p(ctx.snap), ctx.p, _p(uvc), _p(P),
              _p(dA), _p(dEbar), _p(dXin), _p(dX), _p(dE), _p(dflat), _p(dlogit), _p(ds), _p(dvpart), _p(duvc),
              _p(scratch), None if bp is None else bp.queue, _stream())
@@ -284,6 +286,13 @@
     def park(self, leaf, dflat, operands):
         self.keep.append(operands)
         self.installs.append((leaf, dflat))
+
+    def workspace(self, B, N, D, dev):
+        need = _lib.lib().gcgcn_defer_split_ws(self.queue, B, N, D)
+        if need > 0:
+            ws = torch.empty(need, device=dev)
+            self.keep.append(ws)
+            call("gcgcn_defer_workspace", self.queue, _p(ws), need)
 
     def __call__(self):
         with _passes_lock:
diff --git a/include/gcgcn.h b/include/gcgcn.h
--- a/include/gcgcn.h
+++ b/include/gcgcn.h
@@ -83,6 +83,8 @@
 void gcgcn_defer_destroy(void* queue);
 int gcgcn_defer_count(const void* queue);
 int gcgcn_defer_flush(void* queue, void* stream);
+int64_t gcgcn_defer_split_ws(const void* queue, int B, int N, int D);
+int gcgcn_defer_workspace(void* queue, float* ws, int64_t elems);
 
 int gcgcn_graphconv_fwd(int B, int N, int Din, int De, int Dout, const float* X, const float* Ebar, const float* A,
                         const float* We, const float* Wn, const float* bias, float* out, float* T, float* rinv,
@@ -154,6 +156,9 @@
 int gcgcn_debug_edge_plan(int pass, int compact, int B, int N, int D, int ragged, int att, int has_dE, int has_dEbar, int misalign,
                           int parked_tiles, int any_rb, int col_C, int32_t* out);
 
+int gcgcn_debug_carry_ksplit(int n, const int32_t* probs, int64_t rows, int col_C, int64_t ws_have, int64_t* out);
+int gcgcn_debug_carry_stats(int64_t* out);
+
 int gcgcn_debug_attn_plan(int bwd, int N, int D, int H, int hook, int chain_attends, int core_done, int misalign, int32_t* out);
 
 int gcgcn_debug_out_bwd_plan(int fuse, int B, int N, int D, int H, int scratch, int wsum_fwd, int ragged, int odrop, int drop,
```

Result: slower. 63990 docs/s (-3.0%).
